# om-ai-lab/OmChat

Measured on AMD Instinct MI355X. Metric: images/sec prefill + decode tokens/sec, OmChat-13B TP=1/8; p50 TTFT, higher is better.
Workload: dtype bf16

## Files before the change

### include/omchat_hip.h

```cpp
#ifndef OMCHAT_HIP_H
#define OMCHAT_HIP_H
#include <stddef.h>
#include <stdint.h>

#ifdef __cplusplus
extern "C" {
#endif

#define OMCHAT_F16 0
#define OMCHAT_BF16 1
#define OMCHAT_F32 2
#define OMCHAT_PAD_ROW INT32_MIN

typedef struct omchat_ctx omchat_ctx;

typedef struct {
  int v_hidden;
  int v_heads;
  int v_qk_channels;
  int v_mlp;
  int v_layers;
  int v_patch;
  int v_image;
  float v_eps;
// ... 58 lines not shown
#define OMCHAT_CON_MAX_SUPPRESS 1024
#define OMCHAT_CON_MAX_BAD_WORDS 1024
#define OMCHAT_CON_MAX_BAD_WORD_IDS 8192
int omchat_set_constraints(omchat_ctx* ctx, int b, int no_repeat_ngram_size, int min_new_tokens, int min_length, const int32_t* eos_ids, int n_eos,
                           const int32_t* suppress_ids, int n_suppress, const int32_t* begin_suppress_ids, int n_begin_suppress,
                           const int32_t* bad_word_ids, const int32_t* bad_word_offsets, int n_bad_words, const int32_t* prompt_ids,
                           const int32_t* prompt_len, int max_new, void* stream);
#define OMCHAT_FSM_MAX_STATES (1 << 20)
#define OMCHAT_FSM_MAX_EDGES (1 << 26)
#define OMCHAT_FSM_DEAD (-1)
int omchat_fsm_load(omchat_ctx* ctx, int n_states, const int32_t* off, const int32_t* tok, const int32_t* nxt, void* stream);
int omchat_fsm_begin(omchat_ctx* ctx, int b, const int32_t* start_states, int max_new, void* stream);
int omchat_fsm_states(omchat_ctx* ctx, int b, int32_t* out, void* stream);
int omchat_set_guidance(omchat_ctx* ctx, int b, float scale, void* stream);
#define OMCHAT_DOLA_MAX_LAYERS 16
int omchat_set_dola(omchat_ctx* ctx, int b, const int32_t* layers, int k, float relative_top, int norm, void* stream);
int omchat_dola_read(omchat_ctx* ctx, int32_t* out, int rows, int steps);
int omchat_dola_rows(omchat_ctx* ctx, float* out);
int omchat_set_logprobs(omchat_ctx* ctx, int b, int max_new, void* stream);
int omchat_read_logprobs(omchat_ctx* ctx, int b, float* raw, float* processed, int32_t* counts, int max_len);
#define OMCHAT_LP_MAX_TOP 20
#define OMCHAT_LP_MAX_SCORED 32
int omchat_set_logprobs_ex(omchat_ctx* ctx, int b, int max_new, int top_n, const int32_t* score_ids, int n_score, void* stream);
int omchat_read_logprob_extras(omchat_ctx* ctx, int b, float* top_vals, int32_t* top_ids, float* scored, int32_t* counts, int max_len);
int omchat_read_sampling_state(omchat_ctx* ctx, int row, int* step, uint32_t* seen_words);
int omchat_kv_lengths(omchat_ctx* ctx, int32_t* out, int b);
int omchat_kv_rewind(omchat_ctx* ctx, int b, int n, void* stream);

int omchat_beam_begin(omchat_ctx* ctx, int b, int num_beams, float length_penalty, int early_stopping, const int32_t* eos_ids, int n_eos,
                      int max_new, int prompt_tok_len, void* stream);
int omchat_beam_step(omchat_ctx* ctx, const float* logits, int rows, int32_t* next_tokens, int32_t* done_word, void* stream);
int omchat_beam_result(omchat_ctx* ctx, int num_return, int32_t* tokens, int32_t* lengths, float* scores, int max_len);

int omchat_group_begin(omchat_ctx* ctx, int b, int N, int prompt_len, int share, void* stream);
int omchat_group_share_available(omchat_ctx* ctx, int N);

#define OMCHAT_VERIFY_KEEP_ALL 1
#define OMCHAT_VERIFY_SAMPLE 2
int omchat_decode_verify(omchat_ctx* ctx, const int32_t* tokens, int T, float* logits, int32_t* picks,
                         int* n_accept, int flags, void* stream);

int omchat_prefill_extend(omchat_ctx* ctx, const void* embeds, int S_new, int keep, float* logits_last, void* hidden_out, void* stream);
int omchat_extend_attn_form(int S_new, int keep, int Hkv);
int omchat_kv_read(omchat_ctx* ctx, int layer, int which, int pos0, int n, void* out, void* stream);
int omchat_kv_read_row(omchat_ctx* ctx, int row, int layer, int which, int pos0, int n, void* out, void* stream);

int omchat_prefill_suffixes(omchat_ctx* ctx, const void* embeds, int N, int S_max, const int32_t* lengths, int keep, float* logits_last,
                            void* hidden_out, void* stream);
int omchat_suffix_attn_form(int shared, int n_rep);

int omchat_enable_decode_graph(omchat_ctx* ctx, int on);
int omchat_decode_graph_stats(omchat_ctx* ctx, long* steps, long* replays, long* captures);
int omchat_bf16x12_stats(omchat_ctx* ctx, int* roles, long* launches, int* coded);

int omchat_enable_fp8_decode(omchat_ctx* ctx, int on);

int omchat_enable_mxfp4_decode(omchat_ctx* ctx, int mode);

enum omchat_weight_format {
  OMCHAT_WFMT_16 = 0,
  OMCHAT_WFMT_16_PACKED = 1,
  OMCHAT_WFMT_E4M3 = 2,
  OMCHAT_WFMT_MXFP4 = 3,
  OMCHAT_WFMT_MXFP4_PACKED = 4,
  OMCHAT_WFMT_COUNT = 5
};
int omchat_decode_weight_format(int rows, int fp8_on, int mxfp4_mode, int packed16_ready, int geometry_ok, int* x_pack_nb);

int omchat_enable_fp8_kv(omchat_ctx* ctx, int on);
int omchat_enable_fp8_prefill(omchat_ctx* ctx, int on);

#define OMCHAT_PROF_DECODE_GATEUP 0
#define OMCHAT_PROF_PREFILL_GATEUP 1
#define OMCHAT_PROF_VIT_FC1 2
#define OMCHAT_PROF_CATS 3
int omchat_prof_enable(omchat_ctx* ctx, int on);
int omchat_prof_read(omchat_ctx* ctx, int cat, double* total_ms, long* launches, int reset);

int omchat_mha_fwd(const void* qkv, int B, int S, int H, float softmax_scale, int causal, void* out, int dtype, void* stream);
int omchat_mha_fwd_varlen(const void* qkv, int B, int S, int H, int D, const int32_t* seqlens, float softmax_scale, int causal,
                          void* out, int dtype, void* stream);

int omchat_op_gemm(int dtype, const void* A, int lda, const void* W, int ldw, void* C, int ldc, int M, int N, int K,
                   const void* bias, const void* ls, const void* resid, int ldr, int epi, int force_tile, void* stream);
int omchat_op_gemm_fused(int dtype, const void* A, int lda, const void* W, int ldw, void* C, int ldc, int M, int N, int K,
                         const void* bias, const void* ls, const void* resid, int ldr, int epi, int force_tile, const float* row_scale,
                         const float* rs_stats, int rs_ld, int rs_nslots, int rs_dim, float rs_eps,
                         float* stats, int stats_ld, int* nslots, void* stream);
int omchat_op_stats_finish(const float* stats, int ld, int slot0, int nslots, int ngroups, int rows, int dim, float eps, float* out, void* stream);
int omchat_op_row_sumsq(int dtype, const void* x, int ldx, int rows, int H, float* stats, void* stream);
int omchat_op_fold_cols(int dtype, const void* W, const void* n, void* out, int rows, int cols, void* stream);
int omchat_op_vit_knorm_slots(int dtype, void* k, int ld, const void* wk, int rows, int C, int C_total, float eps, const float* stats, int stats_ld,
                              int nslots, float* sumsq_q, void* stream);
int omchat_op_mha_qnorm(int dtype, const void* qkv, int B, int Sq, int H, const float* sumsq, int stride, int dim, const void* wq,
                        float eps, float q_scale, void* out, void* stream);
int omchat_op_gemv_norm(int dtype, const void* X, const void* W, int ldw, void* Y, int N, int K, const void* norm_w, float eps,
                        const void* bias, int epi, int out_f32, void* stream);
int omchat_op_set_tuning(int key, int value);
int omchat_gemm_tune_load(const char* path);
int omchat_gemm_tune_dump(const char* path);
long omchat_gemm_tune_runs(void);
size_t omchat_op_gemm_sk_ws(void);
int omchat_op_gemm_sk(int dtype, const void* A, int lda, const void* W, int ldw, void* C, int ldc, int M, int N, int K,
                      const void* bias, const void* ls, const void* resid, int ldr, int epi, int force_tile, void* ws,
                      size_t ws_bytes, int stream_k, void* stream);
int omchat_op_gemv(int dtype, const void* X, int ldx, const void* W, int ldw, void* Y, int ldy, int b, int N, int K,
                   const void* bias, const void* resid, int ldr, int epi, int out_f32, void* stream);
int omchat_op_gemv_packed(int dtype, const void* X, int ldx, const void* W, int ldw, void* Y, int ldy, int b, int N, int K,
                          const void* bias, int epi, int out_f32, int ksplit, int w_packed, int y_packed, void* stream);
int omchat_op_pack_x(int dtype, const void* X, int ldx, int b, int K, void* out, void* stream);
#define OMCHAT_GEMV_PLAN_INTS 20
int omchat_op_gemv_plan(int dtype, int b, int N, int K, int epi, int ksplit, int flags, int wf, int n_cu, int* out);
int omchat_op_gemv_split_k(int b, int K, int H, int packed, int down);
int omchat_op_gemm_fp8(int dtype, const void* A8, const float* a_scale, const void* W8, const float* w_scale, void* C, int ldc, int M, int N,
                       int K, const void* bias, const void* resid, int ldr, int epi, void* stream);
int omchat_op_quant_rows_fp8(int dtype, const void* x, const void* norm_w, float eps, void* y8, float* scale, int rows, int H, void* stream);
int omchat_op_quant_fp8(int dtype, const void* W, int N, int K, void* W8, float* scale, void* stream);
int omchat_op_gemv_fp8(int dtype, const void* X, const void* W8, const float* scale, void* Y, int N, int K, const void* bias,
                       const void* resid, int epi, int out_f32, int ksplit, void* stream);
int omchat_op_quant_mxfp4(int dtype, const void* W, int N, int K, void* W4, void* S, void* stream);
int omchat_op_gemv_mxfp4(int dtype, const void* X, const void* W4, const void* S, void* Y, int N, int K, const void* bias,
                         const void* resid, int epi, int out_f32, int ksplit, void* stream);
int omchat_op_gemv_mxfp4_norm(int dtype, const void* X, const void* W4, const void* S, void* Y, int N, int K, const void* norm_w, float eps,
                              const void* bias, int epi, int out_f32, void* stream);
int omchat_op_gemv_mxfp4_rows(int dtype, const void* X, int ldx, const void* W4, const void* S, void* Y, int ldy, int b, int N, int K,
                              const void* bias, int epi, int out_f32, int ksplit, void* stream);
int omchat_op_gemv_mxfp4_packed(int dtype, const void* X, int ldx, const void* W4, const void* S, void* Y, int ldy, int b, int N, int K,
                                const void* bias, int epi, int out_f32, int ksplit, int y_packed, void* stream);
int omchat_op_encode_bf16x12(const void* W, int N, int K, void* coded, void* top, void* cnt, void* patch, void* over, void* stream);
int omchat_op_gemv_bf16x12(const void* X, const void* coded, const void* top, const void* cnt, const void* patch, void* Y, int N, int K,
                           const void* norm_w, float eps, const void* resid, int epi, int out_f32, void* stream);
int omchat_op_pack_w(int dtype, const void* W, int ldw, int N, int K, void* out, void* stream);
int omchat_op_pack_w4(const void* W4, const void* S, int N, int K, void* W4P, void* SP, void* stream);
int omchat_op_gemv_prepacked(int dtype, const void* XP, const void* WP, const void* SP, void* Y, int ldy, int b, int N, int K, const void* bias,
                             int epi, int out_f32, int ksplit, int y_packed, void* stream);
int omchat_op_rmsnorm(int dtype, const void* x, const void* w, void* y, int rows, int H, float eps, void* stream);
int omchat_op_resid_rmsnorm(int dtype, void* x, int ldx, const float* part, int ks, const void* w, void* xn, int ldn, int rows, int H,
                            float eps, int pack_nb, void* stream);
int omchat_op_vit_qknorm(int dtype, void* qkv, int ld, const void* wq, const void* wk, int rows, int C, int C_total,
                         float eps, float q_scale, void* stream);
int omchat_op_attn_prefill(int dtype, const void* q, const void* k, const void* v, void* out, int b, int Sq, int Skv,
                           int Hq, int Hkv, const int32_t* kv_len, int causal, int q_pos0, float scale, void* stream);
int omchat_op_attn_prefill_d(int dtype, const void* q, const void* k, const void* v, void* out, int b, int Sq, int Skv,
                             int Hq, int Hkv, int D, const int32_t* kv_len, int causal, int q_pos0, float scale, void* stream);
int omchat_op_layernorm(int dtype, const void* x, const void* w, const void* b, void* y, int rows, int H, float eps, void* stream);
size_t omchat_op_attn_decode_ws(int b, int Hq, int L);
int omchat_op_attn_decode(int dtype, const void* q, const void* k, const void* v, void* out, int b, int Hq, int Hkv,
                          int cap, int L, const int32_t* kv_len, float scale, void* ws, size_t ws_bytes, void* stream);
int omchat_op_attn_verify(int dtype, const void* q, void* k, void* v, void* out, int T, int Hq, int Hkv, int cap, int L, float scale,
                          void* ws, size_t ws_bytes, void* stream);
int omchat_op_attn_verify_tpw(int keys, int Hkv);
size_t omchat_op_attn_extend_ws(int Sq, int Hq, int Hkv, int L);
int omchat_op_attn_extend(int dtype, const void* q, const void* k, const void* v, void* out, int Sq, int Hq, int Hkv, int cap, int L,
                          float scale, void* ws, size_t ws_bytes, void* stream);
size_t omchat_op_attn_shared_ws(int G, int N, int Hq, int Hkv, int P, int L);
int omchat_op_attn_shared(int dtype, const void* q, void* k, void* v, void* out, int G, int N, int Hq, int Hkv, int cap, int P, int L,
                          float scale, void* ws, size_t ws_bytes, void* stream);
int omchat_op_attn_shared_lens(int dtype, const void* q, void* k, void* v, void* out, int G, int N, int Hq, int Hkv, int cap, int P, int L,
                               const int* kv_len, float scale, void* ws, size_t ws_bytes, void* stream);
size_t omchat_op_attn_suffix_ws(int N, int S, int Hq, int Hkv, int P);
int omchat_op_attn_suffix(int dtype, const void* q, const void* k, const void* v, void* out, int N, int S, int Hq, int Hkv, int cap, int P,
                          const int32_t* lengths, int* kv_len_dev, float scale, void* ws, size_t ws_bytes, void* stream);
int omchat_op_attn_verify_append(int dtype, const void* qkv, float theta, void* k, void* v, void* out, int T, int Hq, int Hkv, int cap,
                                 int L, float scale, void* ws, size_t ws_bytes, void* stream);
int omchat_op_attn_decode_kv8(int dtype, const void* q, const void* k8, const void* v8, const float* ks, const float* vs, void* out, int b,
                              int Hq, int Hkv, int cap, int L, const int32_t* kv_len, float scale, void* ws, size_t ws_bytes, void* stream);
int omchat_op_attn_decode_kv8_masked(int dtype, const void* q, const void* k8, const void* v8, const float* ks, const float* vs, void* out, int b,
                                     int Hq, int Hkv, int cap, int L, const unsigned char* key_mask, int64_t mask_sb, float scale, void* ws,
                                     size_t ws_bytes, void* stream);
int omchat_op_attn_merge(int dtype, const float* ws, int nsplit, int q_heads, int rows, const int32_t* kv_len, int L, float scale, void* out,
                         int split_keys, void* stream);
int omchat_op_kv_quant(int dtype, const void* k16, const void* v16, void* k8, void* v8, float* ks, float* vs, int b, int Hkv, int cap,
                       const int32_t* pos_lo, int pos0, const int32_t* len, int max_rows, void* stream);
int omchat_op_attn_decode_kv8_append(int dtype, void* qkv, float theta, void* k8, void* v8, float* ks, float* vs, void* k16, void* v16, void* out,
                                     int b, int Hq, int Hkv, int cap, int L, const int32_t* kv_len, const int32_t* pos, float scale, void* ws,
                                     size_t ws_bytes, void* stream);
int omchat_op_rope_kv(int dtype, void* qkv, int b, int S, int Hq, int Hkv, int pos0, float theta, void* kcache, void* vcache,
                      int cap, void* stream);
int omchat_op_rope_kv_q8(int dtype, void* qkv, int b, int S, int Hq, int Hkv, int pos0, float theta, void* kcache, void* vcache, int cap,
                         void* k8, void* v8, float* ks, float* vs, void* stream);
int omchat_op_argmax(const float* logits, int b, int V, int32_t* out, void* stream);
int omchat_op_attn_prefill_left(int dtype, const void* q, const void* k, const void* v, void* out, int b, int Sq, int Skv, int Hq, int Hkv,
                                const int32_t* kv_len, const int32_t* kv_start, int causal, int q_pos0, float scale, int fill_uniform, void* stream);
int omchat_op_rope_kv_pos(int dtype, void* qkv, int b, int S, int Hq, int Hkv, const int32_t* pos, int pos0, int slot0, int max_pos, float theta,
// ... 99 lines not shown
```

### omchat_amd/_lib.py

```python
import ctypes as C
import os

HERE = os.path.dirname(os.path.abspath(__file__))
LIB_PATH = os.environ.get("OMCHAT_LIB") or os.path.join(HERE, "lib", "libomchat_hip.so")
_lib = None

F16, BF16, F32 = 0, 1, 2
EPI_NONE, EPI_GELU, EPI_LS_RESID, EPI_RESID, EPI_SWIGLU = 0, 1, 2, 3, 4
EPI_F32OUT = 6
EPI_LS_RESID_STATS, EPI_NONE_STATS = 7, 8
PAD_ROW = -(2 ** 31)
PROF_DECODE_GATEUP, PROF_PREFILL_GATEUP, PROF_VIT_FC1 = 0, 1, 2


class OmchatConfig(C.Structure):
    _fields_ = [
        ("v_hidden", C.c_int), ("v_heads", C.c_int), ("v_qk_channels", C.c_int), ("v_mlp", C.c_int), ("v_layers", C.c_int),
        ("v_patch", C.c_int), ("v_image", C.c_int), ("v_eps", C.c_float),
        ("t_hidden", C.c_int), ("t_layers", C.c_int), ("t_heads", C.c_int), ("t_kv_heads", C.c_int), ("t_mlp", C.c_int),
        ("t_vocab", C.c_int), ("t_vocab_total", C.c_int), ("t_eps", C.c_float), ("rope_theta", C.c_float),
        ("max_seq", C.c_int), ("max_batch", C.c_int), ("max_tiles", C.c_int), ("max_prefill_rows", C.c_int), ("dtype", C.c_int),
        ("v_head_dim", C.c_int), ("v_norm_type", C.c_int), ("v_no_qk_norm", C.c_int),
    ]

# ... 39 lines not shown
    "omchat_dola_rows": (_i, [_vp, _vp]),
    "omchat_op_dola_ws": (_sz, [_i, _i, _i]),
    "omchat_op_dola": (_i, [_vp, _i, _i, _i, _i, _f, _vp, _i, _vp, _vp, _sz, _vp]),
    "omchat_kv_lengths": (_i, [_vp, _vp, _i]),
    "omchat_kv_rewind": (_i, [_vp, _i, _i, _vp]),
    "omchat_set_logprobs": (_i, [_vp, _i, _i, _vp]),
    "omchat_read_logprobs": (_i, [_vp, _i, _vp, _vp, _vp, _i]),
    "omchat_set_logprobs_ex": (_i, [_vp, _i, _i, _i, _vp, _i, _vp]),
    "omchat_read_logprob_extras": (_i, [_vp, _i, _vp, _vp, _vp, _vp, _i]),
    "omchat_group_begin": (_i, [_vp, _i, _i, _i, _i, _vp]),
    "omchat_group_share_available": (_i, [_vp, _i]),
    "omchat_beam_begin": (_i, [_vp, _i, _i, _f, _i, _vp, _i, _i, _i, _vp]),
    "omchat_beam_step": (_i, [_vp, _vp, _i, _vp, _vp, _vp]),
    "omchat_beam_result": (_i, [_vp, _i, _vp, _vp, _vp, _i]),
    "omchat_decode_verify": (_i, [_vp, _vp, _i, _vp, _vp, _vp, _i, _vp]),
    "omchat_decode_step_masked": (_i, [_vp, _vp, _i, _vp, _vp, _i, _vp, _vp, _vp]),
    "omchat_masked_decode_begin": (_i, [_vp, _i, _vp, _vp, _i, _i, _vp]),
    "omchat_decode_step_masked_next": (_i, [_vp, _vp, _i, _vp, _vp, _vp]),
    "omchat_fused_status": (_i, [_vp, C.POINTER(C.c_long), C.POINTER(C.c_uint)]),
    "omchat_has_experiments": (_i, []),
    "omchat_set_allreduce_hook": (_i, [_vp, _vp, _vp]),
    "omchat_allreduce_noop": (_i, [_vp, _vp, C.c_size_t, _i, _vp]),
    "omchat_op_gemv_norm": (_i, [_i, _vp, _vp, _i, _vp, _i, _i, _vp, _f, _vp, _i, _i, _vp]),
    "omchat_prof_enable": (_i, [_vp, _i]),
    "omchat_prof_read": (_i, [_vp, _i, C.POINTER(C.c_double), C.POINTER(C.c_long), _i]),
    "omchat_mha_fwd": (_i, [_vp, _i, _i, _i, _f, _i, _vp, _i, _vp]),
    "omchat_mha_fwd_varlen": (_i, [_vp, _i, _i, _i, _i, _vp, _f, _i, _vp, _i, _vp]),
    "omchat_op_gemm": (_i, [_i, _vp, _i, _vp, _i, _vp, _i, _i, _i, _i, _vp, _vp, _vp, _i, _i, _i, _vp]),
    "omchat_op_gemm_fused": (_i, [_i, _vp, _i, _vp, _i, _vp, _i, _i, _i, _i, _vp, _vp, _vp, _i, _i, _i, _vp, _vp, _i, _i, _i, _f, _vp, _i, _vp, _vp]),
    "omchat_op_stats_finish": (_i, [_vp, _i, _i, _i, _i, _i, _i, _f, _vp, _vp]),
    "omchat_op_row_sumsq": (_i, [_i, _vp, _i, _i, _i, _vp, _vp]),
    "omchat_op_fold_cols": (_i, [_i, _vp, _vp, _vp, _i, _i, _vp]),
    "omchat_op_vit_knorm_slots": (_i, [_i, _vp, _i, _vp, _i, _i, _i, _f, _vp, _i, _i, _vp, _vp]),
    "omchat_op_mha_qnorm": (_i, [_i, _vp, _i, _i, _i, _vp, _i, _i, _vp, _f, _f, _vp, _vp]),
    "omchat_ctx_sp_stats": (_i, [_vp, C.POINTER(C.c_long), C.POINTER(C.c_long)]),
    "omchat_op_set_tuning": (_i, [_i, _i]),
    "omchat_gemm_tune_load": (_i, [C.c_char_p]),
    "omchat_gemm_tune_dump": (_i, [C.c_char_p]),
    "omchat_gemm_tune_runs": (C.c_long, []),
    "omchat_op_gemm_sk_ws": (_sz, []),
    "omchat_op_gemm_sk": (_i, [_i, _vp, _i, _vp, _i, _vp, _i, _i, _i, _i, _vp, _vp, _vp, _i, _i, _i, _vp, _sz, _i, _vp]),
    "omchat_op_gemv": (_i, [_i, _vp, _i, _vp, _i, _vp, _i, _i, _i, _i, _vp, _vp, _i, _i, _i, _vp]),
    "omchat_op_gemv_packed": (_i, [_i, _vp, _i, _vp, _i, _vp, _i, _i, _i, _i, _vp, _i, _i, _i, _i, _i, _vp]),
    "omchat_op_pack_x": (_i, [_i, _vp, _i, _i, _i, _vp, _vp]),
    "omchat_op_gemv_plan": (_i, [_i, _i, _i, _i, _i, _i, _i, _i, _i, _vp]),
    "omchat_op_gemv_split_k": (_i, [_i, _i, _i, _i, _i]),
    "omchat_op_gemm_fp8": (_i, [_i, _vp, _vp, _vp, _vp, _vp, _i, _i, _i, _i, _vp, _vp, _i, _i, _vp]),
    "omchat_op_quant_rows_fp8": (_i, [_i, _vp, _vp, _f, _vp, _vp, _i, _i, _vp]),
    "omchat_enable_fp8_decode": (_i, [_vp, _i]),
    "omchat_enable_fp8_kv": (_i, [_vp, _i]),
    "omchat_enable_fp8_prefill": (_i, [_vp, _i]),
    "omchat_enable_decode_graph": (_i, [_vp, _i]),
    "omchat_bf16x12_stats": (_i, [_vp, C.POINTER(_i), C.POINTER(C.c_long), C.POINTER(_i)]),
    "omchat_decode_graph_stats": (_i, [_vp, C.POINTER(C.c_long), C.POINTER(C.c_long), C.POINTER(C.c_long)]),
    "omchat_op_quant_fp8": (_i, [_i, _vp, _i, _i, _vp, _vp, _vp]),
    "omchat_op_gemv_fp8": (_i, [_i, _vp, _vp, _vp, _vp, _i, _i, _vp, _vp, _i, _i, _i, _vp]),
    "omchat_enable_mxfp4_decode": (_i, [_vp, _i]),
    "omchat_decode_weight_format": (_i, [_i, _i, _i, _i, _i, C.POINTER(_i)]),
    "omchat_op_quant_mxfp4": (_i, [_i, _vp, _i, _i, _vp, _vp, _vp]),
    "omchat_op_gemv_mxfp4": (_i, [_i, _vp, _vp, _vp, _vp, _i, _i, _vp, _vp, _i, _i, _i, _vp]),
    "omchat_op_gemv_mxfp4_rows": (_i, [_i, _vp, _i, _vp, _vp, _vp, _i, _i, _i, _i, _vp, _i, _i, _i, _vp]),
    "omchat_op_gemv_mxfp4_packed": (_i, [_i, _vp, _i, _vp, _vp, _vp, _i, _i, _i, _i, _vp, _i, _i, _i, _i, _vp]),
    "omchat_op_pack_w": (_i, [_i, _vp, _i, _i, _i, _vp, _vp]),
    "omchat_op_pack_w4": (_i, [_vp, _vp, _i, _i, _vp, _vp, _vp]),
    "omchat_op_gemv_prepacked": (_i, [_i, _vp, _vp, _vp, _vp, _i, _i, _i, _i, _vp, _i, _i, _i, _i, _vp]),
    "omchat_op_encode_bf16x12": (_i, [_vp, _i, _i, _vp, _vp, _vp, _vp, _vp, _vp]),
    "omchat_op_gemv_bf16x12": (_i, [_vp, _vp, _vp, _vp, _vp, _vp, _i, _i, _vp, _f, _vp, _i, _i, _vp]),
    "omchat_op_gemv_mxfp4_norm": (_i, [_i, _vp, _vp, _vp, _vp, _i, _i, _vp, _f, _vp, _i, _i, _vp]),
    "omchat_op_rmsnorm": (_i, [_i, _vp, _vp, _vp, _i, _i, _f, _vp]),
    "omchat_op_resid_rmsnorm": (_i, [_i, _vp, _i, _vp, _i, _vp, _vp, _i, _i, _i, _f, _i, _vp]),
    "omchat_op_vit_qknorm": (_i, [_i, _vp, _i, _vp, _vp, _i, _i, _i, _f, _f, _vp]),
    "omchat_op_attn_prefill": (_i, [_i, _vp, _vp, _vp, _vp, _i, _i, _i, _i, _i, _vp, _i, _i, _f, _vp]),
    "omchat_op_attn_prefill_d": (_i, [_i, _vp, _vp, _vp, _vp, _i, _i, _i, _i, _i, _i, _vp, _i, _i, _f, _vp]),
    "omchat_op_layernorm": (_i, [_i, _vp, _vp, _vp, _vp, _i, _i, _f, _vp]),
    "omchat_op_attn_decode_ws": (_sz, [_i, _i, _i]),
    "omchat_op_attn_decode": (_i, [_i, _vp, _vp, _vp, _vp, _i, _i, _i, _i, _i, _vp, _f, _vp, _sz, _vp]),
    "omchat_op_attn_verify_tpw": (_i, [_i, _i]),
    "omchat_op_attn_verify": (_i, [_i, _vp, _vp, _vp, _vp, _i, _i, _i, _i, _i, _f, _vp, _sz, _vp]),
    "omchat_op_attn_extend_ws": (_sz, [_i, _i, _i, _i]),
    "omchat_op_attn_shared_ws": (_sz, [_i, _i, _i, _i, _i, _i]),
    "omchat_op_attn_shared": (_i, [_i, _vp, _vp, _vp, _vp, _i, _i, _i, _i, _i, _i, _i, _f, _vp, _sz, _vp]),
    "omchat_op_attn_extend": (_i, [_i, _vp, _vp, _vp, _vp, _i, _i, _i, _i, _i, _f, _vp, _sz, _vp]),
    "omchat_prefill_extend": (_i, [_vp, _vp, _i, _i, _vp, _vp, _vp]),
    "omchat_extend_attn_form": (_i, [_i, _i, _i]),
    "omchat_kv_read": (_i, [_vp, _i, _i, _i, _i, _vp, _vp]),
    "omchat_kv_read_row": (_i, [_vp, _i, _i, _i, _i, _i, _vp, _vp]),
    "omchat_prefill_suffixes": (_i, [_vp, _vp, _i, _i, _vp, _i, _vp, _vp, _vp]),
    "omchat_suffix_attn_form": (_i, [_i, _i]),
    "omchat_op_attn_shared_lens": (_i, [_i, _vp, _vp, _vp, _vp, _i, _i, _i, _i, _i, _i, _i, _vp, _f, _vp, _sz, _vp]),
    "omchat_op_attn_suffix_ws": (_sz, [_i, _i, _i, _i, _i]),
    "omchat_op_attn_suffix": (_i, [_i, _vp, _vp, _vp, _vp, _i, _i, _i, _i, _i, _i, _vp, _vp, _f, _vp, _sz, _vp]),
    "omchat_op_attn_verify_append": (_i, [_i, _vp, _f, _vp, _vp, _vp, _i, _i, _i, _i, _i, _f, _vp, _sz, _vp]),
    "omchat_op_attn_decode_kv8": (_i, [_i, _vp, _vp, _vp, _vp, _vp, _vp, _i, _i, _i, _i, _i, _vp, _f, _vp, _sz, _vp]),
    "omchat_op_attn_decode_kv8_masked": (_i, [_i, _vp, _vp, _vp, _vp, _vp, _vp, _i, _i, _i, _i, _i, _vp, _i64, _f, _vp, _sz, _vp]),
    "omchat_op_attn_merge": (_i, [_i, _vp, _i, _i, _i, _vp, _i, _f, _vp, _i, _vp]),
    "omchat_op_kv_quant": (_i, [_i, _vp, _vp, _vp, _vp, _vp, _vp, _i, _i, _i, _vp, _i, _vp, _i, _vp]),
    "omchat_op_attn_decode_kv8_append": (_i, [_i, _vp, _f, _vp, _vp, _vp, _vp, _vp, _vp, _vp, _i, _i, _i, _i, _i, _vp, _vp, _f, _vp, _sz, _vp]),
    "omchat_op_attn_decode_append": (_i, [_i, _vp, _f, _vp, _vp, _vp, _i, _i, _i, _i, _i, _vp, _vp, _vp, _i64, _i, _f, _vp, _sz, _vp]),
    "omchat_op_rope_kv": (_i, [_i, _vp, _i, _i, _i, _i, _i, _f, _vp, _vp, _i, _vp]),
    "omchat_op_rope_kv_q8": (_i, [_i, _vp, _i, _i, _i, _i, _i, _f, _vp, _vp, _i, _vp, _vp, _vp, _vp, _vp]),
    "omchat_op_argmax": (_i, [_vp, _i, _i, _vp, _vp]),
    "omchat_op_attn_prefill_left": (_i, [_i, _vp, _vp, _vp, _vp, _i, _i, _i, _i, _i, _vp, _vp, _i, _i, _f, _i, _vp]),
    "omchat_op_rope_kv_pos": (_i, [_i, _vp, _i, _i, _i, _i, _vp, _i, _i, _i, _f, _vp, _vp, _i, _vp]),
    "omchat_op_argmax_ld": (_i, [_vp, _i, _i, _i, _vp, _vp, _vp, _vp]),
    "omchat_op_im2col": (_i, [_i, _vp, _vp, _i, _i, _i, _i, _vp]),
    "omchat_op_vit_assemble": (_i, [_i, _vp, _vp, _vp, _vp, _i, _i, _i, _vp]),
    "omchat_op_gather_rows": (_i, [_i, _vp, _vp, _vp, _vp, _i, _i, _vp]),
    "omchat_op_copy_rows": (_i, [_i, _vp, _i64, _vp, _i64, _i, _i, _i, _i, _vp]),
    "omchat_op_tp_finish": (_i, [_i, _vp, _vp, _vp, _vp, _vp, _i, _i, _i, _vp]),
    "omchat_op_resid16_norm": (_i, [_i, _vp, _i, _vp, _i, _vp, _vp, _vp, _i, _i, _i, _f, _vp]),
    "omchat_op_cast_f32": (_i, [_i, _vp, _vp, _i64, _vp]),
    "omchat_op_rmsnorm_ld": (_i, [_i, _vp, _i, _vp, _vp, _i, _i, _i, _f, _i, _vp]),
    "omchat_op_layernorm_ld": (_i, [_i, _vp, _i, _vp, _vp, _vp, _i, _i, _i, _f, _vp]),
    "omchat_op_sample": (_i, [_vp, _i, _i, _u64, _f, _i, C.c_double, _f, _vp, _vp, _i, _vp, _vp, _vp]),
    "omchat_op_token_logprob": (_i, [_vp, _i, _i, _i, _vp, _vp, _f, _f, _vp, _vp, _vp, _vp, _vp, _vp, _vp]),
    "omchat_op_lse_label_ws": (_sz, [_i, _i]),
    "omchat_op_lse_label": (_i, [_i, _vp, _i, _vp, _i, _i, _i, _i, _vp, _vp, _vp, _vp, _sz, _vp]),
    "omchat_op_top_logprobs": (_i, [_vp, _i, _i, _i, _i, _vp, _i, _vp, _vp, _vp, _vp]),
    "omchat_op_sample_filtered": (_i, [_vp, _i, _i, _u64, _f, _i, C.c_double, _f, C.c_double, C.c_double, C.c_double, C.c_double, _vp, _vp, _i,
                                       _vp, _vp, _vp, _vp]),
# ... 87 lines not shown
```

### omchat_amd/csrc/capi.hip

```cpp
#include "kernels.h"
#include <stdlib.h>
#include "../../include/omchat_hip.h"
#include <math.h>
#include <vector>

#define S(x) ((hipStream_t)(x))
#if OMCHAT_EXPERIMENTS
int g_launch_any_order = 0;
#endif

extern "C" int omchat_op_gemm(int dtype, const void* A, int lda, const void* W, int ldw, void* C, int ldc, int M, int N, int K,
                              const void* bias, const void* ls, const void* resid, int ldr, int epi, int force_tile, void* stream) {
  GemmArgs g{A, lda, W, ldw, C, ldc, M, N, K, bias, ls, resid, ldr, epi, force_tile, nullptr, 0, -1};
  return launch_gemm(dtype, g, S(stream));
}

extern "C" int omchat_op_gemm_fused(int dtype, const void* A, int lda, const void* W, int ldw, void* C, int ldc, int M, int N, int K,
                                    const void* bias, const void* ls, const void* resid, int ldr, int epi, int force_tile, const float* row_scale,
                                    const float* rs_stats, int rs_ld, int rs_nslots, int rs_dim, float rs_eps,
                                    float* stats, int stats_ld, int* nslots, void* stream) {
  GemmArgs g{A, lda, W, ldw, C, ldc, M, N, K, bias, ls, resid, ldr, epi, force_tile, nullptr, 0, -1};
  g.row_scale = row_scale; g.stats = stats; g.stats_ld = stats_ld; g.stats_nslots = nslots;
  g.rs_stats = rs_stats; g.rs_ld = rs_ld; g.rs_nslots = rs_nslots; g.rs_dim = rs_dim; g.rs_eps = rs_eps;
  return launch_gemm(dtype, g, S(stream));
// ... 21 lines not shown
  a.V = (const char*)qkv + (size_t)2 * H * 128 * 2; a.v_sb = a.q_sb; a.v_sh = 128; a.v_sr = row;
  a.O = out; a.o_sb = (int64_t)Sq * H * 128; a.o_sh = 128; a.o_sr = (int64_t)H * 128;
  a.batch = B; a.q_heads = H; a.kv_heads = H; a.Sq = Sq; a.Skv = Sq; a.kv_len = nullptr; a.causal = 0; a.q_pos0 = 0;
  a.scale = 1.0f;
  a.qn_sumsq = sumsq; a.qn_stride = stride; a.qn_dim = dim; a.qn_w = wq; a.qn_eps = eps; a.qn_scale = q_scale;
  return launch_attn_prefill(dtype, a, S(stream));
}

extern "C" int omchat_op_set_tuning(int key, int value) {
  const char* allow = getenv("OMCHAT_ALLOW_TUNING");
  if (!allow || allow[0] != '1') {
    omchat_set_error("omchat_op_set_tuning: process-global test / measurement hook; set OMCHAT_ALLOW_TUNING=1 to use it (see include/omchat_hip.h)");
    return 1;
  }
  if (key == 0) { gemm_set_skew(value); return 0; }
  if (key == 1) { gemv_set_force_mfma(value); return 0; }
  if (key == 5) { gemm_set_autotune(value); return 0; }
  if (key == 4) { model_set_ar_min_rows(value); return 0; }
  if (key == 6) { model_set_pack_replica(value); return 0; }
  if (key == 8) { attn_set_v2(value); return 0; }
  if (key == 9) { model_set_fuse_peer_norm(value); return 0; }
  if (key == 10) { attn_set_tpw(value); return 0; }
  if (key == 11) { gemv_set_no_xs(value); return 0; }
  if (key == 12) { attn_set_klds(value); return 0; }
  if (key == 25) { attn_set_dma(value); return 0; }
  if (key == 26) { attn_set_dma_slots(value); return 0; }
  if (key == 27) { attn_set_dma_rot(value); return 0; }
  if (key == 28) { gemv_set_skew(value); return 0; }
  if (key == 29) { model_set_tp_f32(value); return 0; }
  if (key == 30) { attn_set_hsplit(value); return 0; }
  if (key == 33) { attn_set_mha_xcd(value); return 0; }
  if (key == 16) { gemv_set_norm_loop(value); return 0; }
  if (key == 17) { gemv_set_rows_balance(value); return 0; }
  if (key == 19) { attn_set_merge_mid_min(value); return 0; }
  if (key == 21) { attn_set_merge_dg(value); return 0; }
  if (key == 13) { gemm_set_persist(value); return 0; }
  if (key == 14) { model_set_norm_in_gemv(value); return 0; }
  if (key == 22) { model_set_fuse_attn_oproj(value); return 0; }
  if (key == 23) { model_set_decode_layer(value); return 0; }
  if (key == 24) { gemv_set_dyn(value); return 0; }
  if (key == 34) { gemv_set_shard_shapes(value); return 0; }
  if (key == 35) { model_set_shard_as_tp1(value); return 0; }
  if (key == 36) { attn_set_kg(value); return 0; }
  if (key == 37) { gemm_set_wide_store(value); return 0; }
  if (key == 43) { gemm_set_skip_dead(value); return 0; }
  if (key == 44) { model_set_vit_fused(value); return 0; }
  if (key == 45) { model_set_tp_sp(value); return 0; }
  if (key == 46) { attn_set_peel(value); return 0; }
  if (key == 47) { attn_set_kv8_tpw(value); return 0; }
  if (key == 48) { attn_set_kv8_fuse(value); return 0; }
  if (key == 49) { model_set_extend_attn(value); return 0; }
  if (key == 50) { model_set_x12_roles(value); return 0; }
  if (key == 51) { model_set_suffix_attn(value); return 0; }
  if (key == 38) { gemv_set_gu_rr(value); return 0; }
  if (key == 39) { gemv_set_longk_direct(value); return 0; }
  if (key == 40) { norm_set_wave(value); return 0; }
#if OMCHAT_EXPERIMENTS
  if (key == 41) { g_launch_any_order = value; return 0; }
  if (key == 42) { model_set_ao_oproj(value); return 0; }
#endif
  omchat_set_error("omchat_op_set_tuning: unknown key");
  return 1;
}

extern "C" int omchat_allreduce_noop(void*, void*, size_t, int, void*) { return 0; }

extern "C" int omchat_gemm_tune_load(const char* path) { OM_CHECK(path, "null path"); return gemm_tune_load(path); }
extern "C" int omchat_gemm_tune_dump(const char* path) { OM_CHECK(path, "null path"); return gemm_tune_dump(path); }
extern "C" long omchat_gemm_tune_runs(void) { return gemm_tune_runs(); }

extern "C" size_t omchat_op_gemm_sk_ws(void) { return gemm_sk_ws_bytes(); }

extern "C" int omchat_op_gemm_sk(int dtype, const void* A, int lda, const void* W, int ldw, void* C, int ldc, int M, int N, int K,
                                 const void* bias, const void* ls, const void* resid, int ldr, int epi, int force_tile, void* ws,
                                 size_t ws_bytes, int stream_k, void* stream) {
  GemmArgs g{A, lda, W, ldw, C, ldc, M, N, K, bias, ls, resid, ldr, epi, force_tile, ws, ws_bytes, stream_k};
  return launch_gemm(dtype, g, S(stream));
}

extern "C" int omchat_op_gemv(int dtype, const void* X, int ldx, const void* W, int ldw, void* Y, int ldy, int b, int N, int K,
                              const void* bias, const void* resid, int ldr, int epi, int out_f32, void* stream) {
  GemvArgs g{X, ldx, W, ldw, Y, ldy, b, N, K, bias, resid, ldr, epi, out_f32};
  return launch_gemv(dtype, g, S(stream));
}

extern "C" int omchat_op_gemv_norm(int dtype, const void* X, const void* W, int ldw, void* Y, int N, int K, const void* norm_w, float eps,
                                   const void* bias, int epi, int out_f32, void* stream) {
  OM_CHECK(X && W && Y && norm_w, "null argument");
  GemvArgs g{X, K, W, ldw, Y, N, 1, N, K, bias, nullptr, 0, epi, out_f32};
  g.norm_w = norm_w; g.norm_eps = eps;
  return launch_gemv(dtype, g, S(stream));
}

extern "C" int omchat_op_gemv_packed(int dtype, const void* X, int ldx, const void* W, int ldw, void* Y, int ldy, int b, int N, int K,
                                     const void* bias, int epi, int out_f32, int ksplit, int w_packed, int y_packed, void* stream) {
  OM_CHECK(b >= 1 && b <= 32 && K % 64 == 0, "1 <= b <= 32, K % 64 == 0");
  const int NB = b > 16 ? 2 : 1;
  void *xp = nullptr, *wp = nullptr;
  OM_HIP(hipMalloc(&xp, (size_t)NB * 16 * K * 2));
  int rc = launch_pack_x(dtype, X, ldx, b, K, xp, S(stream));
  if (rc == 0 && w_packed) {
    if (hipMalloc(&wp, (size_t)N * K * 2) != hipSuccess) { hipFree(xp); omchat_set_error("hipMalloc failed"); return 2; }
    rc = launch_pack_w(dtype, W, ldw, N, K, wp, S(stream));
  }
  if (rc == 0) {
    GemvArgs g{xp, K, w_packed ? wp : W, ldw, Y, ldy, b, N, K, bias, nullptr, 0, epi, out_f32, ksplit, 0, nullptr, 1, w_packed, y_packed};
    rc = launch_gemv(dtype, g, S(stream));
  }
  hipStreamSynchronize(S(stream));
  hipFree(xp); if (wp) hipFree(wp);
  return rc;
}
extern "C" int omchat_op_pack_x(int dtype, const void* X, int ldx, int b, int K, void* out, void* stream) { return launch_pack_x(dtype, X, ldx, b, K, out, S(stream)); }

extern "C" int omchat_op_gemv_plan(int dtype, int b, int N, int K, int epi, int ksplit, int flags, int wf, int n_cu, int* out) {
  OM_CHECK(out && wf >= WF_16 && wf <= WF_X12, "null out or weight form outside 0..3");
  static const unsigned set[1] = {0};
  GemvArgs a{};
  a.b = b; a.N = N; a.K = K; a.epi = epi; a.ksplit = ksplit;
  a.ldx = K; a.ldy = a.ldr = N; a.ldw = wf == WF_MX4 ? K / 2 : wf == WF_X12 ? K / 2 * 3 : K;
  a.x_packed = flags & 1; a.w_packed = flags >> 1 & 1; a.y_packed = flags >> 2 & 1; a.out_f32 = flags >> 4 & 1; a.force_mfma = flags >> 5 & 1;
  if (flags & 8) a.norm_w = set;
  if (flags & 64) a.resid = set;
  if (wf == WF_E4M3) a.w_scale = (const float*)set;
  if (wf == WF_MX4) a.mx_scale = (const unsigned char*)set;
  if (wf == WF_X12) { a.x12_top = a.x12_cnt = (const unsigned char*)set; a.x12_patch = set; }
  const GemvPlan g = gemv_plan(dtype, a, gemv_tuning(), n_cu > 0 ? n_cu : device_cus());
  if (g.refusal) { omchat_set_error(g.refusal); return 1; }
  const int f[OMCHAT_GEMV_PLAN_INTS] = {g.family, g.wf, g.wpack, g.epi, g.ntile, g.waves, g.unroll, g.nb, g.rr, g.nch, g.norm, g.gx, g.gy, g.block, g.lds,
                                        g.per_wg, (int)g.skew, g.rows_per_wg, g.n5, g.xskew};
  for (int i = 0; i < OMCHAT_GEMV_PLAN_INTS; ++i) out[i] = f[i];
  return 0;
}
extern "C" int omchat_op_gemv_split_k(int b, int K, int H, int packed, int down) { return gemv_split_k(b, K, H, packed != 0, down != 0, gemv_tuning()); }

extern "C" int omchat_op_gemm_fp8(int dtype, const void* A8, const float* a_scale, const void* W8, const float* w_scale, void* C, int ldc, int M,
                                  int N, int K, const void* bias, const void* resid, int ldr, int epi, void* stream) {
  GemmArgs g{A8, K, W8, K, C, ldc, M, N, K, bias, nullptr, resid, ldr, epi, 0, nullptr, 0, -1, 1, a_scale, w_scale};
  return launch_gemm(dtype, g, S(stream));
}
extern "C" int omchat_op_quant_rows_fp8(int dtype, const void* x, const void* norm_w, float eps, void* y8, float* scale, int rows, int H, void* stream) {
  if (norm_w) return launch_rmsnorm_q8(dtype, x, H, norm_w, y8, H, scale, rows, H, eps, S(stream));
  return launch_quant_rows_q8(dtype, x, H, y8, H, scale, rows, H, S(stream));
}

extern "C" int omchat_op_resid_rmsnorm(int dtype, void* x, int ldx, const float* part, int ks, const void* w, void* xn, int ldn, int rows, int H,
                                       float eps, int pack_nb, void* stream) {
  OM_CHECK(x && part, "null argument");
  return launch_resid_rmsnorm(dtype, x, ldx, part, ks, w, xn, ldn, rows, H, eps, S(stream), pack_nb);
}
extern "C" int omchat_op_rmsnorm(int dtype, const void* x, const void* w, void* y, int rows, int H, float eps, void* stream) {
  return launch_rmsnorm(dtype, x, H, w, y, H, rows, H, eps, S(stream));
}

extern "C" int omchat_op_vit_qknorm(int dtype, void* qkv, int ld, const void* wq, const void* wk, int rows, int C, int C_total, float eps,
                                    float q_scale, void* stream) {
  return launch_vit_qknorm(dtype, qkv, ld, wq, wk, rows, C, C_total, eps, q_scale, nullptr, S(stream));
}

extern "C" int omchat_op_attn_prefill(int dtype, const void* q, const void* k, const void* v, void* out, int b, int Sq, int Skv, int Hq,
                                      int Hkv, const int32_t* kv_len, int causal, int q_pos0, float scale, void* stream) {
  AttnArgs a{};
  a.Q = q; a.q_sb = (int64_t)Sq * Hq * 128; a.q_sh = 128; a.q_sr = (int64_t)Hq * 128;
  a.K = k; a.k_sb = (int64_t)Hkv * Skv * 128; a.k_sh = (int64_t)Skv * 128; a.k_sr = 128;
  a.V = v; a.v_sb = a.k_sb; a.v_sh = a.k_sh; a.v_sr = 128;
  a.O = out; a.o_sb = a.q_sb; a.o_sh = 128; a.o_sr = a.q_sr;
  a.batch = b; a.q_heads = Hq; a.kv_heads = Hkv; a.Sq = Sq; a.Skv = Skv; a.kv_len = kv_len; a.causal = causal; a.q_pos0 = q_pos0; a.scale = scale;
  return launch_attn_prefill(dtype, a, S(stream));
}

extern "C" size_t omchat_op_attn_decode_ws(int b, int Hq, int L) { return attn_decode_ws_bytes(b, Hq, L); }

static void bind_dense(AttnOperands& a, const void* q, bool qkv_rows, const void* k, const void* v, void* out, int Hq, int Hkv, int cap, float scale,
                       void* ws, size_t ws_bytes) {
  a.Q = q; a.q_sb = (int64_t)(qkv_rows ? Hq + 2 * Hkv : Hq) * 128; a.q_sh = 128;
  a.K = k; a.k_sb = (int64_t)Hkv * cap * 128; a.k_sh = (int64_t)cap * 128; a.k_sr = 128;
  a.V = v; a.v_sb = a.k_sb; a.v_sh = a.k_sh; a.v_sr = 128;
  a.O = out; a.o_sb = (int64_t)Hq * 128; a.o_sh = 128;
  a.q_heads = Hq; a.kv_heads = Hkv; a.scale = scale; a.ws = (float*)ws; a.ws_bytes = ws_bytes;
// ... 706 lines not shown
  const int NB = b > 16 ? 2 : 1;
  void *xp = nullptr, *wp = nullptr, *sp = nullptr;
  auto drop = [&]() { if (xp) hipFree(xp); if (wp) hipFree(wp); if (sp) hipFree(sp); };
  if (hipMalloc(&xp, (size_t)NB * 16 * K * 2) != hipSuccess || hipMalloc(&wp, (size_t)N * (K / 2)) != hipSuccess ||
      hipMalloc(&sp, (size_t)N * (K / 32)) != hipSuccess) {
    (void)hipGetLastError(); drop(); omchat_set_error("hipMalloc failed"); return 2;
  }
  int rc = launch_pack_x(dtype, X, ldx, b, K, xp, S(stream));
  if (rc == 0) rc = launch_pack_w4(W4, (const unsigned char*)S_, N, K, wp, (unsigned char*)sp, S(stream));
  if (rc == 0) {
    GemvArgs g{xp, K, wp, K / 2, Y, ldy, b, N, K, bias, nullptr, 0, epi, out_f32, ksplit, 0, nullptr, 1, 1, y_packed};
    g.mx_scale = (const unsigned char*)sp;
    rc = launch_gemv(dtype, g, S(stream));
  }
  hipStreamSynchronize(S(stream));
  drop();
  return rc;
}

extern "C" int omchat_op_pack_w(int dtype, const void* W, int ldw, int N, int K, void* out, void* stream) { return launch_pack_w(dtype, W, ldw, N, K, out, S(stream)); }
extern "C" int omchat_op_pack_w4(const void* W4, const void* S_, int N, int K, void* W4P, void* SP, void* stream) {
  return launch_pack_w4(W4, (const unsigned char*)S_, N, K, W4P, (unsigned char*)SP, S(stream));
}
extern "C" int omchat_op_gemv_prepacked(int dtype, const void* XP, const void* WP, const void* SP, void* Y, int ldy, int b, int N, int K, const void* bias,
                                        int epi, int out_f32, int ksplit, int y_packed, void* stream) {
  OM_CHECK(XP && WP && Y, "null argument");
  OM_CHECK(b >= 1 && b <= 32 && K >= 64 && K % 64 == 0 && N >= 16 && N % 16 == 0, "pre-packed GEMV: 1 <= b <= 32, K % 64 == 0, N % 16 == 0");
  GemvArgs g{XP, K, WP, SP ? K / 2 : K, Y, ldy, b, N, K, bias, nullptr, 0, epi, out_f32, ksplit, 0, nullptr, 1, 1, y_packed};
  g.mx_scale = (const unsigned char*)SP;
  return launch_gemv(dtype, g, S(stream));
}

extern "C" int omchat_op_gemv_mxfp4_norm(int dtype, const void* X, const void* W4, const void* S_, void* Y, int N, int K, const void* norm_w,
                                         float eps, const void* bias, int epi, int out_f32, void* stream) {
  OM_CHECK(X && W4 && S_ && Y && norm_w, "null argument");
  OM_CHECK(K % 32 == 0, "MXFP4: K must be a multiple of 32 (one e8m0 scale per 32 consecutive k)");
  GemvArgs g{X, K, W4, K / 2, Y, N, 1, N, K, bias, nullptr, 0, epi, out_f32};
  g.norm_w = norm_w; g.norm_eps = eps;
  g.mx_scale = (const unsigned char*)S_;
  return launch_gemv(dtype, g, S(stream));
}

extern "C" int omchat_op_encode_bf16x12(const void* W, int N, int K, void* coded, void* top, void* cnt, void* patch, void* over, void* stream) {
  return launch_encode_bf16x12(W, K, N, K, coded, (unsigned char*)top, (unsigned char*)cnt, (unsigned*)patch, (int*)over, S(stream));
}
extern "C" int omchat_op_gemv_bf16x12(const void* X, const void* coded, const void* top, const void* cnt, const void* patch, void* Y, int N, int K,
                                      const void* norm_w, float eps, const void* resid, int epi, int out_f32, void* stream) {
  OM_CHECK(X && coded && top && cnt && patch && Y, "null argument");
  GemvArgs g{X, K, coded, K / 2 * 3, Y, N, 1, N, K, nullptr, resid, N, epi, out_f32};
  g.norm_w = norm_w; g.norm_eps = eps;
  g.x12_top = (const unsigned char*)top; g.x12_cnt = (const unsigned char*)cnt; g.x12_patch = (const unsigned*)patch;
  return launch_gemv(OMCHAT_BF16, g, S(stream));
}

extern "C" int omchat_op_attn_prefill_d(int dtype, const void* q, const void* k, const void* v, void* out, int b, int Sq, int Skv, int Hq,
                                        int Hkv, int D, const int32_t* kv_len, int causal, int q_pos0, float scale, void* stream) {
  AttnArgs a{};
  a.Q = q; a.q_sb = (int64_t)Sq * Hq * D; a.q_sh = D; a.q_sr = (int64_t)Hq * D;
  a.K = k; a.k_sb = (int64_t)Hkv * Skv * D; a.k_sh = (int64_t)Skv * D; a.k_sr = D;
  a.V = v; a.v_sb = a.k_sb; a.v_sh = a.k_sh; a.v_sr = D;
  a.O = out; a.o_sb = a.q_sb; a.o_sh = D; a.o_sr = a.q_sr;
  a.batch = b; a.q_heads = Hq; a.kv_heads = Hkv; a.Sq = Sq; a.Skv = Skv; a.kv_len = kv_len; a.causal = causal; a.q_pos0 = q_pos0; a.scale = scale;
  a.head_dim = D;
  return launch_attn_prefill(dtype, a, S(stream));
}

extern "C" int omchat_op_layernorm(int dtype, const void* x, const void* w, const void* b, void* y, int rows, int H, float eps, void* stream) {
  return launch_layernorm(dtype, x, H, w, b, y, H, rows, H, eps, S(stream));
}

extern "C" int omchat_op_attn_prefill_left(int dtype, const void* q, const void* k, const void* v, void* out, int b, int Sq, int Skv, int Hq,
                                           int Hkv, const int32_t* kv_len, const int32_t* kv_start, int causal, int q_pos0, float scale,
                                           int fill_uniform, void* stream) {
  OM_CHECK(q && k && v && out && kv_start, "null argument");
  AttnArgs a{};
  a.Q = q; a.q_sb = (int64_t)Sq * Hq * 128; a.q_sh = 128; a.q_sr = (int64_t)Hq * 128;
  a.K = k; a.k_sb = (int64_t)Hkv * Skv * 128; a.k_sh = (int64_t)Skv * 128; a.k_sr = 128;
  a.V = v; a.v_sb = a.k_sb; a.v_sh = a.k_sh; a.v_sr = 128;
  a.O = out; a.o_sb = a.q_sb; a.o_sh = 128; a.o_sr = a.q_sr;
  a.batch = b; a.q_heads = Hq; a.kv_heads = Hkv; a.Sq = Sq; a.Skv = Skv; a.kv_len = kv_len; a.kv_start = kv_start; a.causal = causal;
  a.q_pos0 = q_pos0; a.scale = scale;
  int rc = launch_attn_prefill(dtype, a, S(stream));
  if (!rc && fill_uniform) rc = launch_attn_uniform_rows(dtype, a, S(stream));
  return rc;
}

extern "C" int omchat_op_rope_kv_pos(int dtype, void* qkv, int b, int Sq, int Hq, int Hkv, const int32_t* pos, int pos0, int slot0, int max_pos,
                                     float theta, void* kcache, void* vcache, int cap, void* stream) {
  OM_CHECK(qkv && kcache && vcache && b >= 1 && Sq >= 1 && Hq >= 1 && Hkv >= 1 && max_pos >= 1 && cap >= 1 && slot0 >= -1, "bad argument");
  if (pos) {
    std::vector<int32_t> hp((size_t)b * Sq);
    OM_HIP(hipStreamSynchronize(S(stream)));
    OM_HIP(hipMemcpy(hp.data(), pos, hp.size() * 4, hipMemcpyDeviceToHost));
    for (int32_t p : hp) {
      OM_CHECK(p >= 0 && p < max_pos, "position outside the RoPE table");
      OM_CHECK(slot0 >= 0 || p < cap, "cache slot exceeds the capacity");
    }
  } else {
    OM_CHECK(pos0 >= 0 && pos0 + Sq <= max_pos, "position outside the RoPE table");
    OM_CHECK(slot0 >= 0 || pos0 + Sq <= cap, "cache slot exceeds the capacity");
  }
  OM_CHECK(slot0 < 0 || slot0 + Sq <= cap, "cache slot exceeds the capacity");
  float* d = rope_table_device(max_pos, theta);
  OM_CHECK(d, "rope table allocation failed");
  RopeArgs r{qkv, (Hq + 2 * Hkv) * 128, b * Sq, Sq, Hq, Hkv, pos, pos0, d, max_pos, kcache, vcache, (int64_t)Hkv * cap * 128, (int64_t)cap * 128};
  r.slot0 = slot0;
// ... 57 lines not shown
```

### omchat_amd/csrc/ctx.h

```cpp
#pragma once
#include "kernels.h"
#include "../../include/omchat_hip.h"
#include <rccl/rccl.h>
#include <algorithm>
#include <string>
#include <unordered_map>
#include <vector>

#define TRY(x) do { int rc_ = (x); if (rc_) return rc_; } while (0)

extern int g_fuse_peer_norm;

enum RouteKind { R_PLAIN = 0, R_GATE = 1, R_UP = 2, R_PATCH = 3 };
struct Route {
  void* dst = nullptr;
  int64_t rows = 0, cols = 0;
  int64_t dst_ld = 0;
  int kind = R_PLAIN;
  bool loaded = false;
  float synth_std = 0.02f, synth_off = 0.f;
};

struct Grown {
  void* p = nullptr; size_t cap = 0;
// ... 77 lines not shown
  bool dola_fresh = false;
  bool dola_on() const { return dola.on; }
  bool guidance_on() const { return gd.on; }
  int pick_rows(int rows) const { return gd.on ? rows / 2 : rows; }
  bool sampling_on() const { return smp.on; }
  bool constraints_on() const { return con.on; }
  bool logprobs_on() const { return lp.on; }
  bool fsm_on() const { return fsm.on; }
  void release() { con_hist.release(); lp_rec.release(); lp_xrec.release(); fsm_mem.release(); fsm_trail.release(); dola_rec.release(); }
};

struct BeamState {
  struct Search { bool on = false; int b = 0, N = 0, KB = 0, max_new = 0, P = 0, es = 0, ns = 1, t = 0; float lp = 1.f; std::vector<int> eos; };
  Search cur;
  Grown state, table, dn, parents, stash;
  bool stash8 = false;
  std::vector<int> hpos, hlen;
  bool on() const { return cur.on; }
  void end() { cur.on = false; }
  void release() { for (Grown* g : {&state, &table, &dn, &parents, &stash}) g->release(); }
};

struct GroupState {
  bool share = false; int b = 0, N = 0, P = 0;
  Grown ws;
  std::vector<int> hpos, hlen;
  bool on() const { return share; }
  void end() { share = false; }
  void release() { ws.release(); }
};

struct omchat_ctx {
  omchat_config c;
  int dt = OMCHAT_BF16;
  int tp_rank = 0, tp_size = 1;
  ncclComm_t comm = nullptr;
  std::vector<void*> allocs;
  size_t bytes = 0;
  std::unordered_map<std::string, Route> routes;

  int v_np = 0, v_ntok = 0, v_Cq = 0, v_kpad = 0, v_hd = 128;
  int t_qdim = 0, t_kvdim = 0, t_qkvdim = 0;

  struct VitLayer { void *ls1, *ls2, *n1, *n2, *n1b, *n2b, *wqkv, *qn, *kn, *wproj, *bproj, *w1, *b1, *w2, *b2; };
  struct DecLayer { void *ln1, *ln2, *wqkv, *bqkv, *wo, *wgu, *wd; };
  enum Proj { P_QKV = 0, P_O = 1, P_GU = 2, P_DOWN = 3, P_LM = 4 };
  struct WRef { void* W = nullptr; int ldw = 0; float* w_scale = nullptr; unsigned char* mx_scale = nullptr; int packed = 0; };
  enum WState { W_ABSENT = 0, W_BUILT, W_STALE, W_UNAVAILABLE };
  struct WTable { std::vector<WRef> e; int state = W_ABSENT; };
  WTable wt[OMCHAT_WFMT_COUNT];
  const WRef* layer_w(int fmt, int layer) const { return &wt[fmt].e[(size_t)layer * 4]; }
  const WRef& lm_w(int fmt) const { return wt[fmt].e.back(); }
  bool built(int fmt) const { return wt[fmt].state == W_BUILT; }
  enum X12Role { X12_GU = 0, X12_DOWN = 1, X12_LM = 2, X12_ROLES = 3 };
  struct X12Ref { void* W = nullptr; unsigned char* top = nullptr; unsigned char* cnt = nullptr; unsigned* patch = nullptr; bool ok = false; };
  struct X12Table { std::vector<X12Ref> e; int state = W_ABSENT; };
  X12Table x12[X12_ROLES];
  int* x12_over = nullptr;
  long x12_launches[X12_ROLES] = {0, 0, 0};
  bool fp8_decode = false;
  int mxfp4_mode = 0;
  void *k8cache = nullptr, *v8cache = nullptr;
  float *ks8 = nullptr, *vs8 = nullptr;
  bool fp8_kv = false, kv8_valid = false, fp8_prefill = false;
  void* tw_q8 = nullptr; float* tw_q8s = nullptr;
  int64_t scale_layer_stride() const { return (int64_t)c.max_batch * c.t_kv_heads * c.max_seq; }
  struct DecodeGraph { hipGraph_t graph = nullptr; hipGraphExec_t exec = nullptr; int cap_len = 0, grp_N = 0, grp_P = 0; const void* grp_ws = nullptr; };
  std::unordered_map<int, DecodeGraph> graphs;
  bool graph_on = false;
  hipStream_t graph_stream = nullptr;
  hipEvent_t graph_ev_in = nullptr, graph_ev_out = nullptr;
  int32_t *d_tok_in = nullptr, *d_tok_out = nullptr;
  long graph_steps = 0, graph_replays = 0, graph_captures = 0;
  void *v_cls = nullptr, *v_pos = nullptr, *v_wpatch = nullptr, *v_bpatch = nullptr;
  std::vector<VitLayer> vl;
  void *p_w0 = nullptr, *p_b0 = nullptr, *p_w2 = nullptr, *p_b2 = nullptr;
  void *t_embed = nullptr, *t_norm = nullptr, *t_lm = nullptr;
  std::vector<DecLayer> dl;
  float* rope = nullptr;

  void *vw_cols = nullptr, *vw_pe = nullptr, *vw_x = nullptr, *vw_x2 = nullptr, *vw_xn = nullptr, *vw_qkv = nullptr, *vw_ao = nullptr,
       *vw_h = nullptr, *vw_feat = nullptr, *vw_proj = nullptr;
  float* vw_sumsq = nullptr;
  float *vw_stats_x = nullptr, *vw_stats_qk = nullptr, *vw_rstd = nullptr;
  int vw_stats_x_ld = 0, vw_stats_qk_ld = 0, vw_stats_x_ld_used = 1;
  struct VitFold { void *wqkv = nullptr, *w1 = nullptr; };
  std::vector<VitFold> vfold;
  bool vfold_stale = true;
  void *tw_x = nullptr, *tw_x2 = nullptr, *tw_xn = nullptr, *tw_qkv = nullptr, *tw_ao = nullptr, *tw_act = nullptr, *tw_last = nullptr;
  float* tw_logits = nullptr;
  void* sk_ws = nullptr; size_t sk_ws_bytes = 0;
  float* tp_f32_ws = nullptr; size_t tp_f32_bytes = 0;
  float* tw_part = nullptr;
  float* tw_attn_ws = nullptr;
  size_t tw_attn_ws_bytes = 0;
  void* fd_ws = nullptr;
  unsigned* fd_err = nullptr;
  unsigned fd_epoch = 0;
  long n_fused_launches = 0;
  void* dl_ws = nullptr;
  long n_layer_launches = 0;
  unsigned long long* dbg_stamps = nullptr;
  unsigned* dyn_ctr = nullptr;
  int *d_pos = nullptr, *d_len = nullptr, *d_idx = nullptr, *d_start = nullptr;
  int* d_verify_n = nullptr;
  PickState pick;
  BeamState beam;
  GroupState group;
  Grown ext_ws;
  Grown score_ws;
  int grow(Grown& g, size_t n) {
    if (n <= g.cap) return 0;
// ... 170 lines not shown
```

### omchat_amd/csrc/gemv.hip

```cpp
#include "kernels.h"
#include "rowdot.h"
#include <type_traits>

namespace {

struct GemvP {
  const void* X; const void* W; void* Y; const void* bias; const void* resid;
  int ldx, ldw, ldy, ldr, b, N, K, out_f32, ksplit;
  const float* w_scale;
  int y_packed;
  const void* norm_w; float norm_eps;
  unsigned* dyn;
  void* y_pack;
  unsigned long long* dbg;
  const unsigned char* mx_s;
  const unsigned char* x12_top;
  const unsigned char* x12_cnt;
  const unsigned* x12_patch;
#if OMCHAT_EXPERIMENTS
  int xskew;
#endif
};
#if OMCHAT_EXPERIMENTS
#define OM_DBG_MIN(slot, cond) do { if (p.dbg && (cond) && threadIdx.x == 0) atomicMax(p.dbg + (slot), ~wall_clock64()); } while (0)
// ... 650 lines not shown
  s.pv = p.x12_patch[row * 32 + (lane & 31)];
}
__device__ __forceinline__ void x12_row_finish(X12Row& s) {
  const int t = __builtin_amdgcn_readfirstlane((int)s.top_raw) - 7;
  s.cnt = __builtin_amdgcn_readfirstlane((int)s.cnt_raw);
  s.pi = 0;
  s.tlo = ((unsigned)((t + 1) & 0x7f) << 8) | ((unsigned)((t + 2) & 0x7f) << 16) | ((unsigned)((t + 3) & 0x7f) << 24);
  s.thi = (unsigned)((t + 4) & 0x7f) | ((unsigned)((t + 5) & 0x7f) << 8) | ((unsigned)((t + 6) & 0x7f) << 16) | ((unsigned)((t + 7) & 0x7f) << 24);
}
__device__ __forceinline__ rw_u32x4 x12_decode(const X12W& w, const X12Row& s) {
  const unsigned n = w.nib;
  const unsigned c0 = n & 0x07070707u, c1 = (n >> 4) & 0x07070707u;
  unsigned h0 = __builtin_amdgcn_perm(s.thi, s.tlo, c0), h1 = __builtin_amdgcn_perm(s.thi, s.tlo, c1);
  h0 |= (n & 0x08080808u) << 4;
  h1 |= n & 0x80808080u;
  rw_u32x4 r;
  r.x = __builtin_amdgcn_perm(h0, w.lo.x, 0x05010400u);
  r.y = __builtin_amdgcn_perm(h0, w.lo.x, 0x07030602u);
  r.z = __builtin_amdgcn_perm(h1, w.lo.y, 0x05010400u);
  r.w = __builtin_amdgcn_perm(h1, w.lo.y, 0x07030602u);
  return r;
}
__device__ __forceinline__ void x12_apply(rw_u32x4& w, unsigned e, int lane) {
  const unsigned k = e >> 16, i = k & 7u, sh = (i & 1u) * 16u;
  const unsigned keep = ~(0xffffu << sh), ins = (e & 0xffffu) << sh;
  const bool mine = lane == (int)((k >> 3) & 63u);
  w.x = (mine && (i >> 1) == 0u) ? ((w.x & keep) | ins) : w.x;
  w.y = (mine && (i >> 1) == 1u) ? ((w.y & keep) | ins) : w.y;
  w.z = (mine && (i >> 1) == 2u) ? ((w.z & keep) | ins) : w.z;
  w.w = (mine && (i >> 1) == 3u) ? ((w.w & keep) | ins) : w.w;
}
template <int G>
__device__ __forceinline__ void x12_group(rw_u32x4 (&wd)[G], const X12W* w, X12Row& s, int chunk0, int nch, int lane) {
#pragma unroll
  for (int i = 0; i < G; ++i) wd[i] = x12_decode(w[i], s);
  while (s.pi < s.cnt) {
    const unsigned e = (unsigned)__builtin_amdgcn_readlane((int)s.pv, s.pi);
    const int ch = (int)(e >> 25) - chunk0;
    if (ch >= G) break;
#pragma unroll
    for (int i = 0; i < G; ++i) if (ch == i) x12_apply(wd[i], e, lane);
    ++s.pi;
  }
  if (chunk0 + G > nch) {
    for (int j = 0; j < s.cnt; ++j) {
      const unsigned e = (unsigned)__builtin_amdgcn_readlane((int)s.pv, j);
      if ((e >> 19) != 0u) break;
#pragma unroll
      for (int i = 0; i < G; ++i) if (chunk0 + i >= nch) x12_apply(wd[i], e, 0);
    }
  }
}

template <typename T, int WF>
__device__ __forceinline__ typename RwW<WF>::type rw_ldw(const GemvP& p, size_t row, int k) {
  if constexpr (WF == WF_X12) return x12_ldw(p, row, k >> 9, (k >> 3) & 63); else
  if constexpr (WF == WF_E4M3) {
    return __builtin_nontemporal_load(reinterpret_cast<const rw_u32x2*>((const unsigned char*)p.W + row * p.ldw + k));
  } else if constexpr (WF == WF_MX4) {
    rw_u32x2 w;
    w.x = __builtin_nontemporal_load(reinterpret_cast<const unsigned*>((const unsigned char*)p.W + row * p.ldw + (k >> 1)));
    w.y = __builtin_nontemporal_load(p.mx_s + row * (size_t)(p.K >> 5) + (k >> 5));
    return w;
  } else {
    return __builtin_nontemporal_load(reinterpret_cast<const rw_u32x4*>((const T*)p.W + row * p.ldw + k));
  }
}
template <typename T, int WF>
__device__ __forceinline__ float rw_dotw(typename RwW<WF>::type w, rw_u32x4 x, float acc) {
  if constexpr (WF == WF_E4M3) return rw_dot8_fp8<T>(w, x, acc);
  else if constexpr (WF == WF_MX4) return fmaf(rw_dot8_fp4<T>(w.x, x), mx_scale_of(w.y), acc);
  else return rw_dot8<T>(w, x, acc);
}

template <typename T, int R> struct RwTail { const T* p0; const T* p1; int idx[R]; float v0[R], v1[R]; };
template <typename T, int R> __device__ __forceinline__ void rw_tail_load(RwTail<T, R>& t) {
#pragma unroll
  for (int r = 0; r < R; ++r) { t.v0[r] = tof(t.p0[t.idx[r]]); t.v1[r] = tof(t.p1[t.idx[r]]); }
}
template <typename T, int R, int NCH, int WF>
__device__ __forceinline__ void rw_rows_q(const GemvP& p, const int (&rows)[R], int k0, int lane, const rw_u32x4 (&xr)[RW_MAXC], float (&acc)[R],
                                          RwTail<T, R>& tail) {
  typename RwW<WF>::type w[R][NCH];
#pragma unroll
  for (int r = 0; r < R; ++r)
#pragma unroll
    for (int c = 0; c < NCH; ++c) {
      int k = k0 + c * 512 + lane * 8;
      k = k < p.K ? k : k0;
      w[r][c] = rw_ldw<T, WF>(p, (size_t)rows[r], k);
    }
  float sc[R];
#pragma unroll
  for (int r = 0; r < R; ++r) sc[r] = WF == WF_E4M3 ? p.w_scale[rows[r]] : 1.f;
  rw_tail_load<T, R>(tail);
#pragma unroll
  for (int r = 0; r < R; ++r) {
    float a = 0.f;
#pragma unroll
    for (int c = 0; c < NCH; ++c) a = rw_dotw<T, WF>(w[r][c], xr[c], a);
#pragma unroll
    for (int o = 32; o > 0; o >>= 1) a += __shfl_xor(a, o, 64);
    acc[r] = WF == WF_E4M3 ? a * sc[r] : a;
  }
}

template <typename T, int R, int N, int WF>
__device__ __forceinline__ void rw_dispatch_q(int nch, const GemvP& p, const int (&rows)[R], int k0, int lane, const rw_u32x4 (&xr)[RW_MAXC],
                                              float (&acc)[R], RwTail<T, R>& tail) {
  if constexpr (N > 0) {
    if (nch == N) rw_rows_q<T, R, N, WF>(p, rows, k0, lane, xr, acc, tail);
    else rw_dispatch_q<T, R, N - 1, WF>(nch, p, rows, k0, lane, xr, acc, tail);
  }
}

template <typename T, int R, int NCH>
__device__ __forceinline__ void rw_rows(const T* W, int ldw, const int (&rows)[R], int k0, int K, int lane, const rw_u32x4 (&xr)[RW_MAXC],
                                        float (&acc)[R], RwTail<T, R>& tail) {
  rw_u32x4 w[R][NCH];
#pragma unroll
  for (int r = 0; r < R; ++r)
#pragma unroll
    for (int c = 0; c < NCH; ++c) {
      int k = k0 + c * 512 + lane * 8;
      k = k < K ? k : k0;
      w[r][c] = __builtin_nontemporal_load(reinterpret_cast<const rw_u32x4*>(W + (size_t)rows[r] * ldw + k));
    }
  rw_tail_load<T, R>(tail);
#pragma unroll
  for (int r = 0; r < R; ++r) {
    float a = 0.f;
#pragma unroll
    for (int c = 0; c < NCH; ++c) a = rw_dot8<T>(w[r][c], xr[c], a);
#pragma unroll
    for (int o = 32; o > 0; o >>= 1) a += __shfl_xor(a, o, 64);
    acc[r] = a;
  }
}

template <typename T, int R, int N>
__device__ __forceinline__ void rw_dispatch(int nch, const T* W, int ldw, const int (&rows)[R], int k0, int K, int lane,
                                            const rw_u32x4 (&xr)[RW_MAXC], float (&acc)[R], RwTail<T, R>& tail) {
  if constexpr (N > 0) {
    if (nch == N) rw_rows<T, R, N>(W, ldw, rows, k0, K, lane, xr, acc, tail);
    else rw_dispatch<T, R, N - 1>(nch, W, ldw, rows, k0, K, lane, xr, acc, tail);
  }
}

template <typename T, int EPI, int RR, int WAVES, int F8>
__device__ __forceinline__ void gemv_rows_body(const GemvP& p) {
  constexpr int R = EPI == EPI_SWIGLU ? 2 * RR : RR;
  constexpr int OUT = RR;
  const int lane = threadIdx.x & 63, wave = threadIdx.x >> 6;
  const T* W = (const T*)p.W;
  if constexpr (EPI == EPI_RESID && WAVES == 7) OM_DBG_MIN(1, blockIdx.x < 8);
  const int nch_all = (p.K + 511) / 512;
  const int c_lo = (int)(((long)nch_all * blockIdx.y) / p.ksplit), c_hi = (int)(((long)nch_all * (blockIdx.y + 1)) / p.ksplit);
  const int nch = c_hi - c_lo, k0 = c_lo * 512;
  rw_u32x4 xr[RW_MAXC];
#pragma unroll
  for (int c = 0; c < RW_MAXC; ++c) {
    const int k = k0 + c * 512 + lane * 8;
    rw_u32x4 z = {0u, 0u, 0u, 0u};
    xr[c] = (c < nch && k < p.K) ? *reinterpret_cast<const rw_u32x4*>((const T*)p.X + k) : z;
  }
// ... 7 lines not shown
        int n = g * RR + (r % RR); n = n < n_out ? n : n_out - 1;
        rows[r] = 32 * (n >> 4) + (n & 15) + (r / RR) * 16;
      } else {
        const int n = g * R + r;
        rows[r] = n < p.N ? n : p.N - 1;
      }
    }
    float acc[R];
    RwTail<T, R> tail;
    {
      constexpr bool plain = EPI != EPI_SWIGLU && EPI != EPI_PARTIAL;
      const bool hb = plain && p.bias, hr = EPI == EPI_RESID && !p.out_f32;
      tail.p0 = hb ? (const T*)p.bias : (const T*)p.X;
      tail.p1 = hr ? (const T*)p.resid : (const T*)p.X;
#pragma unroll
      for (int r = 0; r < R; ++r) {
        const int n = g * OUT + r;
        tail.idx[r] = (hb || hr) ? (n < n_out ? n : n_out - 1) : 0;
      }
      if (!hb) tail.p0 = tail.p1;
      if (!hr) tail.p1 = tail.p0;
    }
    if constexpr (F8 != WF_16) rw_dispatch_q<T, R, RW_MAXC, F8>(nch, p, rows, k0, lane, xr, acc, tail);
    else rw_dispatch<T, R, RW_MAXC>(nch, W, p.ldw, rows, k0, p.K, lane, xr, acc, tail);
    if (lane == 0) {
#pragma unroll
      for (int r = 0; r < OUT; ++r) {
        const int n = g * OUT + r;
        if (n >= n_out) continue;
        if constexpr (EPI == EPI_SWIGLU) {
          const float gt = rnd<T>(acc[r]), up = rnd<T>(acc[r + RR]);
          ((T*)p.Y)[n] = fromf<T>(rnd<T>(silu(gt)) * up);
        } else if constexpr (EPI == EPI_PARTIAL) {
          ((float*)p.Y)[(size_t)blockIdx.y * p.ldy + n] = acc[r];
        } else {
          float y = acc[r] + (p.bias ? tail.v0[r] : 0.f);
          if (p.out_f32) ((float*)p.Y)[n] = y;
          else {
            y = rnd<T>(y);
            if constexpr (EPI == EPI_RESID) y = tail.v1[r] + y;
            ((T*)p.Y)[n] = fromf<T>(y);
          }
        }
      }
    }
  }
  if constexpr (EPI == EPI_RESID && WAVES == 7) OM_DBG_MAX(3, (blockIdx.x & 7) == 0);
}

template <typename T, int EPI, int RR = 4, int WAVES = 4, bool F8 = false>
__global__ __launch_bounds__(WAVES * 64) void gemv_rows_kernel(GemvP p) { gemv_rows_body<T, EPI, RR, WAVES, F8 ? WF_E4M3 : WF_16>(p); }
template <typename T, int EPI, int RR, int WAVES>
__global__ __launch_bounds__(WAVES * 64) void gemv_rows_mx4_kernel(GemvP p) { gemv_rows_body<T, EPI, RR, WAVES, WF_MX4>(p); }

template <typename T, int EPI, int RR, int NCH, int F8, int WAVES>
__device__ __forceinline__ void gemv_rows_norm_body(const GemvP& p) {
  typedef typename V8<T>::type v8;
  constexpr int R = EPI == EPI_SWIGLU ? 2 * RR : RR;
  __shared__ __attribute__((aligned(16))) T xs[NCH * 512];
  __shared__ float red[WAVES];
  const int lane = threadIdx.x & 63, wave = __builtin_amdgcn_readfirstlane(threadIdx.x >> 6);
  const int n_out = EPI == EPI_SWIGLU ? p.N / 2 : p.N;
  int g = blockIdx.x * WAVES + wave;
#if OMCHAT_EXPERIMENTS
  if constexpr (EPI == EPI_SWIGLU && RR == 1 && WAVES == 4) {
    if (p.xskew) {
      const int x = blockIdx.x & 7, j = blockIdx.x >> 3;
      const int base = ((n_out + 3) / 4) / 8;
      const int n_x = base + ((x & 1) ? -p.xskew : p.xskew);
      if (j >= n_x) return;
      g = (x * base + ((x & 1) ? p.xskew : 0) + j) * 4 + wave;
    }
  }
#endif
  if constexpr (EPI == EPI_SWIGLU) OM_DBG_MIN(4, blockIdx.x < 8);
  if constexpr (EPI == EPI_NONE) OM_DBG_MIN(8, blockIdx.x < 8);
  static_assert(WAVES >= 4 && NCH <= 8, "sum-of-squares order: four owner waves, up to two chunks each");
  constexpr int MC = (NCH + WAVES - 1) / WAVES;
  constexpr int SC = (NCH + 3) / 4;
  rw_u32x4 xq[MC], nq[MC], sq[SC];
#pragma unroll
  for (int i = 0; i < MC; ++i) {
    const int c = wave + WAVES * i, k = c * 512 + lane * 8;
    const rw_u32x4 z = {0u, 0u, 0u, 0u};
    const bool ok = c < NCH && k < p.K;
    xq[i] = ok ? *reinterpret_cast<const rw_u32x4*>((const T*)p.X + k) : z;
    nq[i] = ok ? *reinterpret_cast<const rw_u32x4*>((const T*)p.norm_w + k) : z;
  }
#pragma unroll
  for (int i = 0; i < SC; ++i) {
    if constexpr (WAVES == 4) {
      sq[i] = xq[i];
    } else {
      const int c = wave + 4 * i, k = c * 512 + lane * 8;
      const rw_u32x4 z = {0u, 0u, 0u, 0u};
      sq[i] = (wave < 4 && c < NCH && k < p.K) ? *reinterpret_cast<const rw_u32x4*>((const T*)p.X + k) : z;
    }
  }
  int rows[R];
#pragma unroll
  for (int r = 0; r < R; ++r) {
    if constexpr (EPI == EPI_SWIGLU) {
      int n = g * RR + (r % RR); n = n < n_out ? n : n_out - 1;
      rows[r] = 32 * (n >> 4) + (n & 15) + (r / RR) * 16;
    } else {
      const int n = g * R + r;
// ... 29 lines not shown
    if constexpr (F8 == WF_E4M3) {
#pragma unroll
      for (int r = 0; r < R; ++r) e_scale[r] = p.w_scale[rows[r]];
    }
  }
  X12Row xst[F8 == WF_X12 ? R : 1];
  if constexpr (F8 == WF_X12) {
#pragma unroll
    for (int r = 0; r < R; ++r) x12_row_load(xst[r], p, (size_t)rows[r], lane);
  }
  __builtin_amdgcn_sched_barrier(0);
  float ss = 0.f;
#pragma unroll
  for (int i = 0; i < SC; ++i) {
    const v8 xv = __builtin_bit_cast(v8, sq[i]);
#pragma unroll
    for (int j = 0; j < 8; ++j) { const float v = tof(xv[j]); ss += v * v; }
  }
#pragma unroll
  for (int o = 32; o > 0; o >>= 1) ss += __shfl_xor(ss, o, 64);
  if (lane == 0 && wave < 4) red[wave] = ss;
  asm volatile("s_waitcnt lgkmcnt(0)" ::: "memory");
  __builtin_amdgcn_s_barrier();
  float tot = red[0];
#pragma unroll
  for (int w = 1; w < 4; ++w) tot += red[w];
  const float inv = rsqrtf(tot / (float)p.K + p.norm_eps);
#pragma unroll
  for (int i = 0; i < MC; ++i) {
    const int c = wave + WAVES * i;
    if (c < NCH) {
      const v8 xv = __builtin_bit_cast(v8, xq[i]), wv = __builtin_bit_cast(v8, nq[i]);
      v8 o;
#pragma unroll
      for (int j = 0; j < 8; ++j) o[j] = fromf<T>(tof(wv[j]) * rnd<T>(tof(xv[j]) * inv));
      *reinterpret_cast<v8*>(xs + c * 512 + lane * 8) = o;
    }
  }
  asm volatile("s_waitcnt lgkmcnt(0)" ::: "memory");
  __builtin_amdgcn_s_barrier();
  rw_u32x4 xr[NCH];
#pragma unroll
  for (int c = 0; c < NCH; ++c) xr[c] = *reinterpret_cast<const rw_u32x4*>(xs + c * 512 + lane * 8);
  __builtin_amdgcn_sched_barrier(0);
  float acc[R];
#pragma unroll
  for (int r = 0; r < R; ++r) {
    float a = 0.f;
    if constexpr (F8 == WF_X12) x12_row_finish(xst[r]);
#pragma unroll
    for (int c = 0; c < NCH; ++c) {
      if constexpr (F8 != WF_X12) a = rw_dotw<T, F8>(w[r][c], xr[c], a);
    }
    if constexpr (F8 == WF_X12) {
      constexpr int G0 = NCH < 4 ? NCH : 4, G1 = NCH - G0;
      {
        rw_u32x4 wd[G0];
        x12_group<G0>(wd, &w[r][0], xst[r], 0, NCH, lane);
#pragma unroll
        for (int c = 0; c < G0; ++c) a = rw_dot8<T>(wd[c], xr[c], a);
      }
      if constexpr (G1 > 0) {
        rw_u32x4 wd[G1];
        x12_group<G1>(wd, &w[r][G0], xst[r], G0, NCH, lane);
#pragma unroll
        for (int c = 0; c < G1; ++c) a = rw_dot8<T>(wd[c], xr[G0 + c], a);
      }
    }
#pragma unroll
    for (int o = 32; o > 0; o >>= 1) a += __shfl_xor(a, o, 64);
    if constexpr (F8 == WF_E4M3) a *= e_scale[r];
    acc[r] = a;
  }
  if (lane == 0) {
#pragma unroll
    for (int r = 0; r < RR; ++r) {
      const int n = g * RR + r;
      if (n >= n_out) continue;
      if constexpr (EPI == EPI_SWIGLU) {
        const float gt = rnd<T>(acc[r]), up = rnd<T>(acc[r + RR]);
        ((T*)p.Y)[n] = fromf<T>(rnd<T>(silu(gt)) * up);
      } else {
        const float y = acc[r] + e_bias[r];
        if (p.out_f32) ((float*)p.Y)[n] = y;
        else ((T*)p.Y)[n] = fromf<T>(y);
      }
    }
  }
  if constexpr (EPI == EPI_SWIGLU) { OM_DBG_MAX(5, blockIdx.x + 64 >= gridDim.x); OM_DBG_MAX(16 + (blockIdx.x & 7), blockIdx.x + 512 >= gridDim.x); }
  if constexpr (EPI == EPI_NONE) OM_DBG_MAX(9, (blockIdx.x & 7) == 0);
}

template <typename T, int EPI, int RR, int NCH, bool F8, int WAVES = 4>
__global__ __launch_bounds__(WAVES * 64) void gemv_rows_norm_kernel(GemvP p) { gemv_rows_norm_body<T, EPI, RR, NCH, F8 ? WF_E4M3 : WF_16, WAVES>(p); }
template <typename T, int EPI, int RR, int NCH, int WAVES = 4>
__global__ __launch_bounds__(WAVES * 64) void gemv_rows_norm_mx4_kernel(GemvP p) { gemv_rows_norm_body<T, EPI, RR, NCH, WF_MX4, WAVES>(p); }
template <typename T, int EPI, int RR, int NCH>
__global__ __launch_bounds__(256) void gemv_rows_norm_x12_kernel(GemvP p) { gemv_rows_norm_body<T, EPI, RR, NCH, WF_X12, 4>(p); }

template <typename T, int EPI, int NCH, int F8>
__device__ __forceinline__ void gemv_rows_norm_loop_body(const GemvP& p, int per_wg, unsigned skew) {
  typedef typename V8<T>::type v8;
  constexpr int R = EPI == EPI_SWIGLU ? 2 : 1;
  __shared__ __attribute__((aligned(16))) T xs[NCH * 512];
  __shared__ float red[4];
  const int lane = threadIdx.x & 63, wave = __builtin_amdgcn_readfirstlane(threadIdx.x >> 6);
  const int n_out = EPI == EPI_SWIGLU ? p.N / 2 : p.N;
  int o0 = blockIdx.x * per_wg, o1 = o0 + per_wg < n_out ? o0 + per_wg : n_out;
  if constexpr (EPI == EPI_SWIGLU) OM_DBG_MIN(4, blockIdx.x < 8);
  if (skew) {
    const int l = blockIdx.x & 7;
    int pre = 0;
    for (int i = 0; i < l; ++i) pre += per_wg + (int)((skew >> (4 * i)) & 15u) - 8;
    o0 = (blockIdx.x >> 3) * 8 * per_wg + pre;
    o1 = o0 + per_wg + (int)((skew >> (4 * l)) & 15u) - 8;
    o1 = o1 < n_out ? o1 : n_out;
  }
  typedef typename RwW<F8>::type wreg_t;
  auto row_of = [&](int n, int r) { return EPI == EPI_SWIGLU ? 32 * (n >> 4) + (n & 15) + r * 16 : n; };
  auto load_w = [&](wreg_t (&w)[R][NCH], int n) {
#pragma unroll
    for (int r = 0; r < R; ++r) {
      const size_t row = (size_t)row_of(n, r);
#pragma unroll
      for (int c = 0; c < NCH; ++c) {
        int k = c * 512 + lane * 8;
        k = k < p.K ? k : 0;
        w[r][c] = rw_ldw<T, F8>(p, row, k);
      }
    }
  };
  wreg_t wa[R][NCH], wb[R][NCH], wc[R][NCH];
  const int u0 = o0 + wave;
  if (u0 < o1) load_w(wa, u0);
  if (u0 + 4 < o1) load_w(wb, u0 + 4);
  if (u0 + 8 < o1) load_w(wc, u0 + 8);
  constexpr int MC = (NCH + 3) / 4;
  rw_u32x4 xq[MC], nq[MC];
#pragma unroll
  for (int i = 0; i < MC; ++i) {
    const int c = wave + 4 * i, k = c * 512 + lane * 8;
    const rw_u32x4 z = {0u, 0u, 0u, 0u};
    const bool ok = c < NCH && k < p.K;
    xq[i] = ok ? *reinterpret_cast<const rw_u32x4*>((const T*)p.X + k) : z;
    nq[i] = ok ? *reinterpret_cast<const rw_u32x4*>((const T*)p.norm_w + k) : z;
  }
  __builtin_amdgcn_sched_barrier(0);
  float ss = 0.f;
#pragma unroll
  for (int i = 0; i < MC; ++i) {
    const v8 xv = __builtin_bit_cast(v8, xq[i]);
// ... 541 lines not shown
    }
  }
  g.block = g.nch = 0;
  return false;
}
}

#define OM_NEED(cond, text) do { if (!(cond)) { g.refusal = text; return g; } } while (0)
GemvPlan gemv_plan(int dtype, const GemvArgs& a, const GemvTuning& t, int n_cu) {
  GemvPlan g{};
  OM_NEED(a.b >= 1 && a.b <= 32, "launch_gemv: batch must be 1..32 per call");
  OM_NEED(!a.x_packed || !a.w_scale, "launch_gemv: packed x: 16-bit or MXFP4 weights");
  OM_NEED(!(a.x_packed && a.mx_scale) || (a.w_packed && a.K % 64 == 0), "launch_gemv: packed x with MXFP4 weights: the packed MXFP4 replica (w_packed), K % 64 == 0");
  OM_NEED(!(a.w_scale && a.mx_scale), "launch_gemv: one weight format per launch: e4m3 (w_scale) or MXFP4 (mx_scale)");
  OM_NEED(!a.w_packed || (a.x_packed && a.N % 16 == 0), "launch_gemv: packed W needs packed x and N % 16 == 0");
  OM_NEED(!a.y_packed || (a.x_packed && a.epi == EPI_SWIGLU), "launch_gemv: packed y: SwiGLU epilogue of the packed kernel only");
  if (a.mx_scale) OM_NEED(a.K % 32 == 0 && a.ldw % 4 == 0 && a.ldx % 8 == 0, "launch_gemv: MXFP4 weights: K % 32 == 0 (one e8m0 scale per 32 k), ldw (bytes) % 4, ldx % 8");
  else OM_NEED(a.K % 64 == 0 && a.ldw % 8 == 0 && a.ldx % 8 == 0, "launch_gemv: K % 64, ldw % 8, ldx % 8");
  OM_NEED((!a.w_scale && !(a.mx_scale && !a.x_packed)) || a.b == 1, "launch_gemv: fp8 / MXFP4 weights: batch 1 only (MXFP4 at b > 1: packed x and the packed MXFP4 replica)");
  OM_NEED(a.epi == EPI_NONE || a.epi == EPI_RESID || a.epi == EPI_SWIGLU || a.epi == EPI_PARTIAL, "launch_gemv: bad epilogue");
  OM_NEED(a.ksplit <= 1 || a.epi == EPI_PARTIAL, "launch_gemv: ksplit > 1 only with EPI_PARTIAL (fp32 slices)");
  OM_NEED(a.ksplit <= (a.K + 63) / 64, "launch_gemv: ksplit exceeds the number of 64-wide K chunks");
  OM_NEED(a.epi != EPI_RESID || a.resid, "launch_gemv: resid missing");
  OM_NEED(a.epi != EPI_SWIGLU || a.N % 32 == 0, "launch_gemv: SwiGLU needs N % 32 == 0");
  OM_NEED(!(a.out_f32 && a.epi != EPI_NONE), "launch_gemv: fp32 output only with EPI_NONE");
  OM_NEED(dtype == OMCHAT_F16 || dtype == OMCHAT_BF16, "launch_gemv: bad dtype");
  const int ks = a.ksplit > 1 ? a.ksplit : 1;
  const bool mfma = a.force_mfma || t.force_mfma;
  g.epi = a.epi; g.gy = 1;
  g.wf = a.x12_top ? WF_X12 : a.mx_scale ? WF_MX4 : a.w_scale ? WF_E4M3 : WF_16;
  OM_NEED(!(a.norm_w && a.x_packed) || (a.w_packed && ks == 1 && (a.K >> 6) == 56 && a.epi == EPI_SWIGLU && a.N % 32 == 0 && !t.no_xs),
          "launch_gemv: the in-register RMSNorm on packed x exists for the x-stationary gate|up form only (packed W, K = 3584, no split-K)");
  OM_NEED(!(a.epi == EPI_RESID && a.x_packed) || (a.w_packed && ks == 1 && (a.K >> 6) == 56 && a.N % 16 == 0 && a.N / 16 <= n_cu && !t.no_xs),
          "launch_gemv: the batched residual epilogue exists for the x-stationary form only (packed W, K = 3584, N / 16 <= CUs, no split-K)");
  if (a.x_packed) {
    g.nb = a.b > 16 ? 2 : 1;
    if (g.wf == WF_X12) g.wf = WF_16;
    OM_NEED(!(a.mx_scale && (a.norm_w || a.epi == EPI_RESID)), "launch_gemv: the batched norm-in-GEMV / residual forms read 16-bit weights only (no MXFP4 instantiation)");
    OM_NEED(OMCHAT_EXPERIMENTS || !(a.norm_w || a.epi == EPI_RESID), "launch_gemv: the batched norm-in-GEMV / residual forms need a -DOMCHAT_EXPERIMENTS=1 build");
    if (plan_xs(g, a, ks, t, n_cu)) return g;
    OM_NEED(!a.norm_w, "launch_gemv: packed-x RMSNorm form: gate|up shape outside the x-stationary launch (N / 32 >= 4 CUs)");
    g.family = GF_PK; g.wpack = a.w_packed != 0; g.ntile = 2; g.waves = 8; g.unroll = 4;
    if (a.epi == EPI_PARTIAL) {
      const int cps = cdiv(a.K >> 6, ks);
      if ((t.shard & 2) && cps <= 32) { g.ntile = 1; g.unroll = cps <= 8 ? 1 : 2; }
      else if (a.K / ks >= 1536) { g.ntile = 4; g.waves = 4; g.unroll = 2; }
    } else if (a.epi == EPI_NONE && a.N >= 32768) { g.ntile = 4; g.waves = 4; }
    g.gx = cdiv(cdiv(a.N, 16), g.ntile); g.gy = ks; g.block = 64 * g.waves;
    return g;
  }
  if (a.x12_top) {
    const bool ok = dtype == OMCHAT_BF16 && a.b == 1 && !a.w_packed && ks == 1 && a.K >= 512 && a.K % 512 == 0 &&
                    a.ldw == a.K / 2 * 3 && a.x12_cnt && a.x12_patch && !a.w_scale && !a.mx_scale && !mfma;
    const bool norm = ok && a.norm_w && (a.epi == EPI_SWIGLU || a.epi == EPI_NONE) && a.K <= RW_MAXC * 512;
    const bool longk = ok && !a.norm_w && a.epi == EPI_RESID && !a.out_f32 && a.K > RW_MAXC * 512 && a.K <= 32768;
    OM_NEED(norm || longk, "launch_gemv: bf16x12 weights: bf16, b == 1, K % 512 == 0, and norm_w with EPI_SWIGLU / EPI_NONE (K <= 4096) or EPI_RESID on 4096 < K <= 32768");
    if (longk) plan_longk(g, a, t, n_cu);
    else { g.rr = rows_per_wave(a, WF_X12, t, n_cu); plan_rows_norm(g, a, t, n_cu); }
    return g;
  }
  if (a.b == 1 && a.epi == EPI_RESID && ks == 1 && !a.out_f32 && a.K > RW_MAXC * 512 && a.K % 8 == 0 && a.K <= 32768 && (!mfma || a.mx_scale)) {
    plan_longk(g, a, t, n_cu);
    return g;
  }
  const bool rows_ok = a.b == 1 && cdiv(cdiv(a.K, 512), ks) <= RW_MAXC;
  OM_NEED(!a.norm_w || (rows_ok && ks == 1 && !mfma && (a.epi == EPI_NONE || a.epi == EPI_SWIGLU)),
          "launch_gemv: the in-register RMSNorm needs the whole-row batch-1 form without split-K (K <= 4096), epilogue NONE / SWIGLU");
  OM_NEED(!(a.w_scale || a.mx_scale) || rows_ok, "launch_gemv: fp8 / MXFP4 weights need b == 1 and <= 8 chunks of 512 per K slice");
  if (rows_ok && (a.w_scale || a.mx_scale || !mfma)) {
    g.rr = rows_per_wave(a, g.wf, t, n_cu);
    if (a.norm_w) plan_rows_norm(g, a, t, n_cu);
    else plan_rows(g, a, ks, t, n_cu);
    return g;
  }
  g.family = GF_MFMA; g.nb = a.b > 16 ? 2 : 1; g.waves = 8; g.unroll = 4;
  g.ntile = a.epi == EPI_SWIGLU || (a.epi == EPI_NONE && (g.nb == 2 || a.N >= 16384)) ? 2 : 1;
  if (g.nb == 1 && a.epi == EPI_PARTIAL && a.K / 64 / ks <= 32) { g.waves = 4; g.unroll = 8; }
  if (g.nb == 1 && a.epi == EPI_NONE) g.unroll = 8;
  g.gx = cdiv(a.N, 16 * g.ntile); g.gy = ks; g.block = 64 * g.waves;
  return g;
}
#undef OM_NEED

int gemv_split_k(int b, int K, int H, bool packed, bool down, const GemvTuning& t) {
  if (b == 1) { const int nch = cdiv(K, 512); return nch >= 16 ? std::min(DEC_KS_MAX, nch) : std::max(1, std::min(3, nch)); }
  if (!down && packed && K == 3584) return 2;
  if ((t.shard & 2) && K / 64 <= 64) return std::max(1, std::min(DEC_KS_MAX, (K / 64) / 16));
  return std::max(1, std::min(DEC_KS_MAX, std::min(K / 64, (down ? 3 : 1) * cdiv(512, cdiv(H, 16)))));
}

namespace {
template <auto KERNEL, typename... A>
int launch_k(const GemvPlan& g, hipStream_t s, const A&... args) {
  hipLaunchKernelGGL(KERNEL, dim3(g.gx, g.gy), dim3(g.block), (size_t)g.lds, s, args...);
  return 0;
}
template <auto KERNEL, typename... A>
int launch_k_lds64(const GemvPlan& g, hipStream_t s, const A&... args) {
  static PerDeviceOnce set;
  if (set.first()) OM_HIP(hipFuncSetAttribute((const void*)KERNEL, hipFuncAttributeMaxDynamicSharedMemorySize, 64 * 1024));
  return launch_k<KERNEL>(g, s, args...);
}
template <int... V, typename F>
int with_int(int v, F&& f) {
  int rc = -1;
  (void)((v == V ? (rc = f(std::integral_constant<int, V>{}), true) : false) || ...);
  return rc;
}
#define IV(c) decltype(c)::value
constexpr bool rows_rr(int epi, int rr, bool q) {
  return epi == EPI_NONE ? rr == 1 || rr == (q ? 8 : 4) : epi == EPI_RESID ? rr == 1 || rr == 4 : epi == EPI_SWIGLU ? rr == 4 || (rr == 1 && !q) : rr == 4;
}
constexpr bool norm_rr(int epi, int rr, bool q) { return epi == EPI_NONE ? rr == 2 || rr == 4 : q ? rr == 1 || rr == 2 || rr == 4 : rr <= 3; }

template <typename T>
int gemv_launch(const GemvPlan& g, const GemvP& p, hipStream_t s) {
  switch (g.family) {
    case GF_MFMA:
#define OM_MFMA(NT_, EPI_, WV_, UN_, NB_)                                                                  \
  if (g.ntile == NT_ && g.epi == EPI_ && g.waves == WV_ && g.unroll == UN_ && g.nb == NB_)                 \
    return launch_k<gemv_kernel<T, NT_, EPI_, WV_, UN_, false, NB_>>(g, s, p)
      OM_MFMA(1, EPI_PARTIAL, 8, 4, 2); OM_MFMA(2, EPI_SWIGLU, 8, 4, 2); OM_MFMA(1, EPI_RESID, 8, 4, 2); OM_MFMA(2, EPI_NONE, 8, 4, 2);
      OM_MFMA(1, EPI_PARTIAL, 4, 8, 1); OM_MFMA(1, EPI_PARTIAL, 8, 4, 1); OM_MFMA(2, EPI_SWIGLU, 8, 4, 1); OM_MFMA(1, EPI_RESID, 8, 4, 1);
      OM_MFMA(2, EPI_NONE, 8, 8, 1); OM_MFMA(1, EPI_NONE, 8, 8, 1);
#undef OM_MFMA
      return -1;
    case GF_PK:
#define OM_PK(NT_, EPI_, WV_, UN_)                                                                         \
  if (g.ntile == NT_ && g.epi == EPI_ && g.waves == WV_ && g.unroll == UN_)                                \
    return with_int<1, 2>(g.nb, [&](auto NB) {                                                             \
      if (g.wf == WF_MX4) return launch_k<gemv_pk_mx4_kernel<T, NT_, EPI_, WV_, UN_, IV(NB)>>(g, s, p);      \
      if (g.wpack) return launch_k<gemv_pk_kernel<T, NT_, EPI_, WV_, UN_, IV(NB), true>>(g, s, p);           \
      return launch_k<gemv_pk_kernel<T, NT_, EPI_, WV_, UN_, IV(NB), false>>(g, s, p);                       \
    })
      OM_PK(2, EPI_SWIGLU, 8, 4); OM_PK(1, EPI_PARTIAL, 8, 1); OM_PK(1, EPI_PARTIAL, 8, 2); OM_PK(4, EPI_PARTIAL, 4, 2); OM_PK(2, EPI_PARTIAL, 8, 4);
      OM_PK(4, EPI_NONE, 4, 4); OM_PK(2, EPI_NONE, 8, 4);
#undef OM_PK
      return -1;
    case GF_XS:
      return with_int<1, 2>(g.nb, [&](auto NB) {
#if OMCHAT_EXPERIMENTS
        if (g.epi == EPI_RESID) return launch_k<gemv_xs_kernel<T, EPI_RESID, IV(NB), 7>>(g, s, p);
        if (g.norm) return launch_k<gemv_xs_kernel<T, EPI_SWIGLU, IV(NB), 7, true>>(g, s, p);
#endif
        return with_int<EPI_SWIGLU, EPI_NONE>(g.epi, [&](auto EPI) {
          if (g.wf == WF_MX4) return launch_k<gemv_xs_mx4_kernel<T, IV(EPI), IV(NB), 7>>(g, s, p);
          return launch_k<gemv_xs_kernel<T, IV(EPI), IV(NB), 7>>(g, s, p);
        });
      });
    case GF_XS_SPLIT:
      return with_int<1, 2>(g.nb, [&](auto NB) {
        if (g.wf == WF_MX4) return launch_k<gemv_xs_split_mx4_kernel<T, IV(NB)>>(g, s, p, g.n5);
        return launch_k<gemv_xs_split_kernel<T, IV(NB)>>(g, s, p, g.n5);
      });
    case GF_ROWS:
      return with_int<EPI_NONE, EPI_RESID, EPI_SWIGLU, EPI_PARTIAL>(g.epi, [&](auto EPI) {
        return with_int<1, 4, 8>(g.rr, [&](auto RR) {
          auto wf = [&](auto WAVES) {
            if (rows_rr(IV(EPI), IV(RR), true)) {
              if (g.wf == WF_MX4) return launch_k<gemv_rows_mx4_kernel<T, IV(EPI), IV(RR), IV(WAVES)>>(g, s, p);
              if (g.wf == WF_E4M3) return launch_k<gemv_rows_kernel<T, IV(EPI), IV(RR), IV(WAVES), true>>(g, s, p);
            }
            if constexpr (IV(RR) != 8) if (rows_rr(IV(EPI), IV(RR), false) && g.wf == WF_16) return launch_k<gemv_rows_kernel<T, IV(EPI), IV(RR), IV(WAVES), false>>(g, s, p);
            return -1;
          };
          if constexpr (IV(EPI) == EPI_RESID && IV(RR) == 1) if (g.waves == 7) return wf(std::integral_constant<int, 7>{});
          return wf(std::integral_constant<int, 4>{});
        });
      });
    case GF_ROWS_NORM:
      return with_int<EPI_SWIGLU, EPI_NONE>(g.epi, [&](auto EPI) {
        return with_int<1, 2, 3, 4, 5, 6, 7, 8>(g.nch, [&](auto NCH) {
          if (g.wf == WF_X12) {
            constexpr int RR = IV(EPI) == EPI_SWIGLU ? 1 : 4;
            if constexpr (std::is_same<T, bf16>::value) if (g.rr == RR) return launch_k<gemv_rows_norm_x12_kernel<bf16, IV(EPI), RR, IV(NCH)>>(g, s, p);
            return -1;
          }
          if constexpr (IV(EPI) == EPI_NONE && IV(NCH) >= 4) if (g.waves == 9 && g.rr == 1) {
            if (g.wf == WF_MX4) return launch_k<gemv_rows_norm_mx4_kernel<T, IV(EPI), 1, IV(NCH), 9>>(g, s, p);
            return g.wf == WF_E4M3 ? launch_k<gemv_rows_norm_kernel<T, IV(EPI), 1, IV(NCH), true, 9>>(g, s, p) : launch_k<gemv_rows_norm_kernel<T, IV(EPI), 1, IV(NCH), false, 9>>(g, s, p);
          }
          return with_int<1, 2, 3, 4>(g.rr, [&](auto RR) {
            if constexpr (IV(RR) != 3) if (norm_rr(IV(EPI), IV(RR), true)) {
              if (g.wf == WF_MX4) return launch_k<gemv_rows_norm_mx4_kernel<T, IV(EPI), IV(RR), IV(NCH)>>(g, s, p);
              if (g.wf == WF_E4M3) return launch_k<gemv_rows_norm_kernel<T, IV(EPI), IV(RR), IV(NCH), true>>(g, s, p);
            }
            if (norm_rr(IV(EPI), IV(RR), false) && g.wf == WF_16) return launch_k<gemv_rows_norm_kernel<T, IV(EPI), IV(RR), IV(NCH), false>>(g, s, p);
            return -1;
          });
        });
      });
    case GF_ROWS_NORM_LOOP:
      return with_int<EPI_SWIGLU, EPI_NONE>(g.epi, [&](auto EPI) {
        return with_int<4, 5, 6, 7, 8>(g.nch, [&](auto NCH) {
          if (g.wf == WF_MX4) return launch_k<gemv_rows_norm_loop_mx4_kernel<T, IV(EPI), IV(NCH)>>(g, s, p, g.per_wg, g.skew);
          return g.wf == WF_E4M3 ? launch_k<gemv_rows_norm_loop_kernel<T, IV(EPI), IV(NCH), true>>(g, s, p, g.per_wg, g.skew) : launch_k<gemv_rows_norm_loop_kernel<T, IV(EPI), IV(NCH), false>>(g, s, p, g.per_wg, g.skew);
        });
      });
    case GF_ROWS_LONGK:
      if (g.wf == WF_X12) {
        if constexpr (std::is_same<T, bf16>::value) return launch_k_lds64<gemv_rows_longk_x12_kernel<T>>(g, s, p, g.rows_per_wg);
        return -1;
      }
      if (g.wf == WF_MX4) return launch_k_lds64<gemv_rows_longk_mx4_kernel<T>>(g, s, p, g.rows_per_wg);
      return g.wf == WF_E4M3 ? launch_k_lds64<gemv_rows_longk_kernel<T, true>>(g, s, p, g.rows_per_wg) : launch_k_lds64<gemv_rows_longk_kernel<T, false>>(g, s, p, g.rows_per_wg);
#if OMCHAT_EXPERIMENTS
    case GF_ROWS_NORM_DYN:
      return with_int<EPI_SWIGLU, EPI_NONE>(g.epi, [&](auto EPI) {
        return with_int<4, 5, 6, 7, 8>(g.nch, [&](auto NCH) {
          if (g.wf == WF_MX4) return launch_k<gemv_rows_norm_dyn_mx4_kernel<T, IV(EPI), IV(NCH)>>(g, s, p);
          return g.wf == WF_E4M3 ? launch_k<gemv_rows_norm_dyn_kernel<T, IV(EPI), IV(NCH), true>>(g, s, p) : launch_k<gemv_rows_norm_dyn_kernel<T, IV(EPI), IV(NCH), false>>(g, s, p);
        });
      });
    case GF_ROWS_LONGK_DIRECT:
      if (g.wf == WF_MX4) return launch_k<gemv_rows_longk_direct_mx4_kernel<T>>(g, s, p);
      return g.wf == WF_E4M3 ? launch_k<gemv_rows_longk_direct_kernel<T, true>>(g, s, p) : launch_k<gemv_rows_longk_direct_kernel<T, false>>(g, s, p);
#endif
  }
  return -1;
}
}

const GemvTuning& gemv_tuning() { return g_tune; }
void gemv_set_force_mfma(int v) { g_tune.force_mfma = v; }
int gemv_get_force_mfma() { return g_tune.force_mfma; }
void gemv_set_no_xs(int v) { g_tune.no_xs = v; }
void gemv_set_shard_shapes(int v) { g_tune.shard = v; }
int gemv_get_shard_shapes() { return g_tune.shard; }
void gemv_set_norm_loop(int v) { g_tune.norm_loop = v; }
void gemv_set_gu_rr(int v) { if (v >= 16) g_tune.gu_rr8 = v / 16; else g_tune.gu_rr = v; }
void gemv_set_dyn(int v) { g_tune.dyn = v; }
void gemv_set_longk_direct(int v) { g_tune.longk_direct = v; }
void gemv_set_skew(int v) { g_tune.skew = (unsigned)v; }
void gemv_set_rows_balance(int v) { g_tune.rows_balance = v; }
int gemv_x12_default_forms() {
  return ((g_tune.norm_loop & 1) == 0 && g_tune.gu_rr == 1 && g_tune.skew == 0u ? 1 : 0) | (g_tune.longk_direct == 0 ? 2 : 0) | ((g_tune.norm_loop & 8) == 0 ? 4 : 0);
}

namespace {
template <typename T>
__global__ __launch_bounds__(256) void quant_fp8_rows_kernel(const T* __restrict__ W, int ldw, int N, int K, unsigned char* __restrict__ W8, int ldq,
                                                             float* __restrict__ scale) {
  const int lane = threadIdx.x & 63, n = blockIdx.x * 4 + (threadIdx.x >> 6);
  if (n >= N) return;
  const T* w = W + (size_t)n * ldw;
  float m = 0.f;
  for (int k = lane * 8; k < K; k += 512) {
    const typename V8<T>::type v = ld8<T>(w + k);
#pragma unroll
    for (int j = 0; j < 8; ++j) m = fmaxf(m, fabsf(tof(v[j])));
  }
#pragma unroll
  for (int o = 32; o > 0; o >>= 1) m = fmaxf(m, __shfl_xor(m, o, 64));
  const float sc = m > 0.f ? m / 448.0f : 1.0f;
  if (lane == 0) scale[n] = sc;
  for (int k = lane * 8; k < K; k += 512) {
    const typename V8<T>::type v = ld8<T>(w + k);
    float f[8];
#pragma unroll
    for (int j = 0; j < 8; ++j) f[j] = tof(v[j]) / sc;
    int lo = 0, hi = 0;
    lo = __builtin_amdgcn_cvt_pk_fp8_f32(f[0], f[1], lo, false);
    lo = __builtin_amdgcn_cvt_pk_fp8_f32(f[2], f[3], lo, true);
    hi = __builtin_amdgcn_cvt_pk_fp8_f32(f[4], f[5], hi, false);
    hi = __builtin_amdgcn_cvt_pk_fp8_f32(f[6], f[7], hi, true);
    rw_u32x2 o2 = {(unsigned)lo, (unsigned)hi};
    *reinterpret_cast<rw_u32x2*>(W8 + (size_t)n * ldq + k) = o2;
  }
}
}

int launch_quant_fp8_rows(int dtype, const void* W, int ldw, int N, int K, void* W8, int ld8, float* scale, hipStream_t s) {
  OM_CHECK(K % 8 == 0 && ldw % 8 == 0 && ld8 % 8 == 0, "K, ldw, ld8 must be multiples of 8");
  if (dtype == OMCHAT_F16) hipLaunchKernelGGL(quant_fp8_rows_kernel<f16>, dim3(cdiv(N, 4)), dim3(256), 0, s, (const f16*)W, ldw, N, K, (unsigned char*)W8, ld8, scale);
  else if (dtype == OMCHAT_BF16) hipLaunchKernelGGL(quant_fp8_rows_kernel<bf16>, dim3(cdiv(N, 4)), dim3(256), 0, s, (const bf16*)W, ldw, N, K, (unsigned char*)W8, ld8, scale);
  else { omchat_set_error("launch_quant_fp8_rows: bad dtype"); return 1; }
  OM_LAUNCH_CHECK();
  return 0;
}

namespace {
template <typename T>
__global__ __launch_bounds__(256) void quant_mxfp4_rows_kernel(const T* __restrict__ W, int ldw, int N, int K, unsigned char* __restrict__ W4, int ld4,
                                                               unsigned char* __restrict__ S) {
  const int lane = threadIdx.x & 63, n = blockIdx.x * 4 + (threadIdx.x >> 6);
  if (n >= N) return;
  const T* w = W + (size_t)n * ldw;
  for (int k = lane * 8; k < K; k += 512) {
    const typename V8<T>::type v = ld8<T>(w + k);
// ... 230 lines not shown
```

### omchat_amd/csrc/kernels.h

```cpp
#pragma once
#ifndef OMCHAT_EXPERIMENTS
#define OMCHAT_EXPERIMENTS 0
#endif
#include "common.h"
#if OMCHAT_EXPERIMENTS
#include <hip/hip_ext.h>
extern int g_launch_any_order;
#undef hipLaunchKernelGGL
#define hipLaunchKernelGGL(kernelName, numBlocks, numThreads, memPerBlock, streamId, ...)                                                      \
  do {                                                                                                                                         \
    if (g_launch_any_order)                                                                                                                    \
      hipExtLaunchKernelGGL((kernelName), dim3(numBlocks), dim3(numThreads), (memPerBlock), (streamId), nullptr, nullptr, hipExtAnyOrderLaunch, \
                            __VA_ARGS__);                                                                                                      \
    else                                                                                                                                       \
      hipLaunchKernelGGLInternal((kernelName), numBlocks, numThreads, memPerBlock, streamId, __VA_ARGS__);                                     \
  } while (0)
#endif

enum {
  EPI_NONE = 0,
  EPI_GELU = 1,
  EPI_LS_RESID = 2,
  EPI_RESID = 3,
  EPI_SWIGLU = 4,
// ... 5 lines not shown
};
struct GemmArgs {
  const void* A; int lda;
  const void* W; int ldw;
  void* C; int ldc;
  int M, N, K;
  const void* bias;
  const void* ls;
  const void* resid;
  int ldr;
  int epi;
  int force_tile;
  void* sk_ws; size_t sk_ws_bytes;
  int stream_k;
  int f8;
  const float* a_scale; const float* w_scale;
  const float* row_scale = nullptr;
  const float* rs_stats = nullptr; int rs_ld = 0, rs_nslots = 0, rs_dim = 0; float rs_eps = 0.f;
  float* stats = nullptr; int stats_ld = 0; int* stats_nslots = nullptr;
  const int* lse_labels = nullptr; float* lse_tgt = nullptr;
};
int launch_gemm(int dtype, const GemmArgs& a, hipStream_t stream);
int launch_stats_finish(const float* stats, int ld, int slot0, int nslots, int ngroups, int rows, int dim, float eps, float* out, hipStream_t s);
int launch_row_sumsq(int dtype, const void* x, int ldx, int rows, int H, float* stats, hipStream_t s);
size_t gemm_sk_ws_bytes();
void gemm_set_skew(int v);
void gemm_set_persist(int v);
void gemm_set_wide_store(int v);
void gemm_set_skip_dead(int v);

struct GemvArgs {
  const void* X; int ldx;
  const void* W; int ldw;
  void* Y; int ldy;
  int b, N, K;
  const void* bias;
  const void* resid; int ldr;
  int epi;
  int out_f32;
  int ksplit;
  int force_mfma;
  const float* w_scale;
  int x_packed;
  int w_packed;
  int y_packed;
  const void* norm_w; float norm_eps;
  void* dyn_ctr = nullptr;
  void* y_pack = nullptr;
  unsigned long long* dbg = nullptr;
  const unsigned char* mx_scale = nullptr;
  const unsigned char* x12_top = nullptr;
  const unsigned char* x12_cnt = nullptr;
  const unsigned* x12_patch = nullptr;
};
int launch_encode_bf16x12(const void* W, int ldw, int N, int K, void* coded, unsigned char* top, unsigned char* cnt, unsigned* patch, int* over,
                          hipStream_t stream);
int launch_pack_x(int dtype, const void* X, int ldx, int b, int K, void* out, hipStream_t s);
int launch_pack_w(int dtype, const void* W, int ldw, int N, int K, void* out, hipStream_t s);
int launch_pack_w4(const void* W4, const unsigned char* S, int N, int K, void* W4P, unsigned char* SP, hipStream_t s);
int launch_gemv(int dtype, const GemvArgs& a, hipStream_t stream);
struct GemvTuning {
  int force_mfma = 0, no_xs = 0, shard = 15, norm_loop = 0, gu_rr = 1, gu_rr8 = 1, dyn = 0, longk_direct = 0, rows_balance = 1;
  unsigned skew = 0;
};
const GemvTuning& gemv_tuning();
enum GemvFamily { GF_MFMA = 0, GF_PK, GF_XS, GF_XS_SPLIT, GF_ROWS, GF_ROWS_NORM, GF_ROWS_NORM_LOOP, GF_ROWS_LONGK, GF_ROWS_NORM_DYN, GF_ROWS_LONGK_DIRECT };
constexpr int WF_16 = 0, WF_E4M3 = 1, WF_MX4 = 2, WF_X12 = 3;
struct GemvPlan {
  const char* refusal;
  int family, wf, wpack, epi, ntile, waves, unroll, nb, rr, nch, norm;
  int gx, gy, block, lds;
  int per_wg; unsigned skew;
  int rows_per_wg;
  int n5;
  int xskew;
};
GemvPlan gemv_plan(int dtype, const GemvArgs& a, const GemvTuning& t, int n_cu);
constexpr int DEC_KS_MAX = 8;
int gemv_split_k(int b, int K, int H, bool packed, bool down, const GemvTuning& t);
int launch_gemv_wait(int dtype, const GemvArgs& a, const unsigned* flags, unsigned epoch, int nflags, unsigned* err, int mode, hipStream_t s);
int launch_quant_fp8_rows(int dtype, const void* W, int ldw, int N, int K, void* W8, int ld8, float* scale, hipStream_t stream);
int launch_quant_mxfp4_rows(int dtype, const void* W, int ldw, int N, int K, void* W4, int ld4, unsigned char* S, hipStream_t stream);
void gemv_set_force_mfma(int v);
int gemv_get_force_mfma();
void gemm_set_autotune(int v);
int gemm_tune_load(const char* path);
int gemm_tune_dump(const char* path);
long gemm_tune_runs();
void model_set_ar_min_rows(int v);
void model_set_tp_f32(int v);
void model_set_pack_replica(int v);
void model_set_norm_in_gemv(int v);
void model_set_vit_fused(int v);
void model_set_tp_sp(int v);
int launch_fold_cols(int dtype, const void* W, const void* n, void* out, int rows, int cols, hipStream_t s);

int launch_layernorm(int dtype, const void* x, int ldx, const void* w, const void* b, void* y, int ldy, int rows, int H, float eps, hipStream_t stream);
int launch_rmsnorm(int dtype, const void* x, int ldx, const void* w, void* y, int ldy, int rows, int H, float eps, hipStream_t s, int pack_nb = 0);
int launch_rmsnorm_q8(int dtype, const void* x, int ldx, const void* w, void* y8, int ldy, float* scale, int rows, int H, float eps, hipStream_t s);
int launch_quant_rows_q8(int dtype, const void* x, int ldx, void* y8, int ldy, float* scale, int rows, int H, hipStream_t s);
int launch_resid_rmsnorm(int dtype, void* x, int ldx, const float* part, int ks, const void* w, void* xn, int ldn, int rows, int H, float eps,
                         hipStream_t s, int pack_nb = 0);
int launch_resid16_norm(int dtype, void* x, int ldx, const void* y, int ldy, const void* w, const void* b, void* xn, int ldn, int rows, int H, float eps,
                        hipStream_t s);
int launch_vit_qknorm(int dtype, void* qkv, int ld, const void* wq, const void* wk, int rows, int C, int C_total,
                      float eps, float q_scale, const float* sumsq_in, hipStream_t s, int only_k = 0);
int launch_vit_qk_sumsq(int dtype, const void* qkv, int ld, int rows, int C, float* sumsq_out, hipStream_t s);
int launch_vit_knorm_slots(int dtype, void* k, int ld, const void* wk, int rows, int C, int C_total, float eps, const float* stats, int stats_ld, int nslots,
                           float* sumsq_q, hipStream_t s);
struct AttnArgs {
  const void* Q; int64_t q_sb, q_sh, q_sr;
  const void* K; int64_t k_sb, k_sh, k_sr;
  const void* V; int64_t v_sb, v_sh, v_sr;
  void* O; int64_t o_sb, o_sh, o_sr;
  int batch, q_heads, kv_heads;
  int Sq, Skv;
  const int* kv_len;
  const int* kv_start;
  int causal;
  int q_pos0;
  float scale;
  int head_dim;
  const float* qn_sumsq = nullptr; int qn_stride = 0, qn_dim = 0; const void* qn_w = nullptr; float qn_eps = 0.f, qn_scale = 1.f;
};
int launch_attn_prefill(int dtype, const AttnArgs& a, hipStream_t s);
int launch_attn_uniform_rows(int dtype, const AttnArgs& a, hipStream_t s);
void attn_set_v2(int v);
void model_set_fuse_peer_norm(int v);
void attn_set_tpw(int v);
void attn_set_klds(int v);
void attn_set_dma(int v);
void attn_set_dma_slots(int v);
void attn_set_dma_rot(int v);
void attn_set_hsplit(int v);
void attn_set_mha_xcd(int v);
void attn_set_kg(int v);
void attn_set_peel(int v);
void attn_set_kv8_tpw(int v);
void attn_set_kv8_fuse(int v);
void model_set_extend_attn(int v);
void model_set_x12_roles(int v);
void model_set_suffix_attn(int v);
int gemv_x12_default_forms();
bool attn_decode_kv8_fuses_rope(int batch, int kv_heads, int L, bool masked);
void attn_set_merge_mid_min(int v);
void attn_set_merge_dg(int v);
void gemv_set_norm_loop(int v);
void gemv_set_dyn(int v);
void gemv_set_skew(int v);
void gemv_set_rows_balance(int v);
void gemv_set_no_xs(int v);
void gemv_set_shard_shapes(int v);
void gemv_set_gu_rr(int v);
void gemv_set_longk_direct(int v);
void norm_set_wave(int v);
void model_set_ao_oproj(int v);
int gemv_get_shard_shapes();

struct AttnOperands {
  const void* Q; int64_t q_sb, q_sh;
  const void* K; int64_t k_sb, k_sh, k_sr;
  const void* V; int64_t v_sb, v_sh, v_sr;
  void* O; int64_t o_sb, o_sh;
  int q_heads, kv_heads;
  float scale;
  float* ws; size_t ws_bytes;
  const float* rope; int rope_max;
  const void* k_new; const void* v_new; int64_t new_sb;
  int o_pack_nb;
};

struct AttnDecodeArgs : AttnOperands {
  int batch;
  int L;
  const int* kv_len;
  const int* pos;
  const float* k_scale; const float* v_scale; int64_t scale_sb, scale_sh;
  void* k16_w = nullptr; void* v16_w = nullptr;
  const unsigned char* key_mask; int64_t mask_sb;
  unsigned* done_flags = nullptr; unsigned done_epoch = 0; int done_mode = 0;
  unsigned long long* done_dbg = nullptr;
};
int launch_kv_quant(int dtype, const void* kc, const void* vc, void* k8, void* v8, float* ks, float* vs, int b, int kv_heads, int64_t c_sb, int64_t c_sh,
                    int64_t s_sb, int64_t s_sh, const int* pos_lo, int pos0, const int* len, int max_rows, hipStream_t s);
size_t attn_decode_ws_bytes(int batch, int q_heads, int max_len);
int launch_attn_decode(int dtype, const AttnDecodeArgs& a, hipStream_t s);
int launch_attn_merge(int dtype, const float* ws, int nsplit, int q_heads, int rows, const int* kv_len, int L, float scale, void* O, int split_keys,
                      hipStream_t s);

enum AttnBlockMode { ATTN_VERIFY = 0, ATTN_EXTEND, ATTN_SHARED, ATTN_SUFFIX };
struct AttnBlockArgs : AttnOperands {
  int mode;
  int G, N, S, P, L;
  const int* kv_len;
};
// ... 207 lines not shown
```

### omchat_amd/csrc/model.hip

```cpp
#include "ctx.h"
#include <limits.h>
#include <math.h>
#include <string.h>
#include <algorithm>
#include <functional>
#include <string>
#include <unordered_map>
#include <vector>

static thread_local std::string g_err;
void omchat_set_error(const std::string& s) { g_err = s; }
extern "C" const char* omchat_last_error(void) { return g_err.c_str(); }
extern "C" const char* omchat_version(void) { return "omchat_hip 0.1 (gfx950)"; }

namespace {

__global__ void cast_from_f32_f16(const float* s, f16* d, int64_t n) {
  for (int64_t i = (int64_t)blockIdx.x * blockDim.x + threadIdx.x; i < n; i += (int64_t)gridDim.x * blockDim.x) d[i] = (f16)s[i];
}
__global__ void cast_from_f32_bf16(const float* s, bf16* d, int64_t n) {
  for (int64_t i = (int64_t)blockIdx.x * blockDim.x + threadIdx.x; i < n; i += (int64_t)gridDim.x * blockDim.x) d[i] = (bf16)s[i];
}
__global__ void add_positions_kernel(int* pos, int b, int d) {
  const int i = threadIdx.x;
// ... 845 lines not shown
  OM_HIP(hipMemcpyAsync(P.dola_hid, xf, (size_t)b * H * 2, hipMemcpyDeviceToDevice, s));
  TRY(launch_rmsnorm(ctx->dt, P.dola_hid, H, ctx->t_norm, P.dola_hid, H, P.dola.norm ? n : b, H, c.t_eps, s));
  TRY(lm_head_rows(ctx, P.dola_hid, n, P.dola_logits, s, ctx->lm_w(OMCHAT_WFMT_16)));
  if (logits) OM_HIP(hipMemcpyAsync(logits, P.dola_logits, (size_t)b * c.t_vocab * 4, hipMemcpyDeviceToDevice, s));
  P.dola_fresh = true;
  return 0;
}
static void* dola_slot(omchat_ctx* ctx, int j) { return (char*)ctx->pick.dola_hid + (size_t)(1 + j) * ctx->pick.dola.b * ctx->c.t_hidden * 2; }

static int build_replica(omchat_ctx* ctx, int fmt) {
  omchat_ctx::WTable& T = ctx->wt[fmt];
  if (T.state == omchat_ctx::W_BUILT) return 0;
  const bool f8 = fmt == OMCHAT_WFMT_E4M3, mx = fmt == OMCHAT_WFMT_MXFP4, mxp = fmt == OMCHAT_WFMT_MXFP4_PACKED, p16 = fmt == OMCHAT_WFMT_16_PACKED;
  if (f8 || mx) OM_CHECK(omchat_weights_missing(ctx) == 0, "load the weights before quantising them");
  if (mx) OM_CHECK(ctx->c.t_hidden % 32 == 0 && ctx->t_qdim % 32 == 0 && ctx->c.t_mlp % 32 == 0,
                   "MXFP4 decode: every streamed K (hidden_size, heads x 128, intermediate_size) must be a multiple of 32");
  if (mxp) TRY(build_replica(ctx, OMCHAT_WFMT_MXFP4));
  const std::vector<omchat_ctx::WRef>& src = ctx->wt[mxp ? OMCHAT_WFMT_MXFP4 : OMCHAT_WFMT_16].e;
  if (T.e.empty()) {
    std::vector<omchat_ctx::WRef> fresh(src.size());
    std::vector<void**> slots;
    std::vector<size_t> sizes;
    for (size_t j = 0; j < fresh.size(); ++j) {
      const size_t N = entry_shape(ctx, j).N, K = entry_shape(ctx, j).K;
      omchat_ctx::WRef& r = fresh[j];
      r.ldw = (int)(mx || mxp ? K / 2 : K);
      r.packed = p16 || mxp;
      slots.push_back(&r.W); sizes.push_back(p16 ? N * K * 2 : f8 ? N * K : N * (K / 2));
      if (f8) { slots.push_back((void**)&r.w_scale); sizes.push_back(N * 4); }
      if (mx || mxp) { slots.push_back((void**)&r.mx_scale); sizes.push_back(N * (K / 32)); }
    }
    if (ctx->alloc_group(slots, sizes)) {
      if (p16) { T.state = omchat_ctx::W_UNAVAILABLE; return 0; }
      if (mxp) omchat_set_error("omchat_enable_mxfp4_decode: the packed MXFP4 replica of mode 2 does not fit in device memory (hipMalloc failed)");
      return 2;
    }
    T.e.swap(fresh);
  }
  for (size_t j = 0; j < T.e.size(); ++j) {
    const int N = entry_shape(ctx, j).N, K = entry_shape(ctx, j).K;
    const omchat_ctx::WRef& w = src[j]; const omchat_ctx::WRef& r = T.e[j];
    if (f8) TRY(launch_quant_fp8_rows(ctx->dt, w.W, K, N, K, r.W, K, r.w_scale, nullptr));
    else if (mx) TRY(launch_quant_mxfp4_rows(ctx->dt, w.W, K, N, K, r.W, K / 2, r.mx_scale, nullptr));
    else if (mxp) TRY(launch_pack_w4(w.W, w.mx_scale, N, K, r.W, r.mx_scale, nullptr));
    else TRY(launch_pack_w(ctx->dt, w.W, K, N, K, r.W, nullptr));
  }
  OM_HIP(hipDeviceSynchronize());
  T.state = omchat_ctx::W_BUILT;
  return 0;
}

int g_x12_roles = 7;
void model_set_x12_roles(int v) { g_x12_roles = v & 7; }

static int x12_step_mask(const omchat_ctx* ctx, int rows, int fmt) {
  if (rows != 1 || fmt != OMCHAT_WFMT_16 || ctx->dt != OMCHAT_BF16 || ctx->tp_size != 1) return 0;
  return g_x12_roles & gemv_x12_default_forms();
}

static int build_x12(omchat_ctx* ctx, int role) {
  omchat_ctx::X12Table& T = ctx->x12[role];
  if (T.state == omchat_ctx::W_BUILT || T.state == omchat_ctx::W_UNAVAILABLE) return 0;
  const omchat_config& c = ctx->c;
  const int H = c.t_hidden, It = c.t_mlp, L = c.t_layers;
  const bool lm = role == omchat_ctx::X12_LM, down = role == omchat_ctx::X12_DOWN;
  const size_t N = lm ? c.t_vocab : down ? H : 2 * (size_t)It, K = down ? It : H, n = lm ? 1 : L;
  const bool k_ok = K % 512 == 0 && (down ? (K > 4096 && K <= 32768) : K <= 4096);
  if (!k_ok || omchat_weights_missing(ctx) != 0) { if (!k_ok) T.state = omchat_ctx::W_UNAVAILABLE; return 0; }
  if (T.e.empty()) {
    std::vector<omchat_ctx::X12Ref> fresh(n);
    std::vector<void**> slots;
    std::vector<size_t> sizes;
    for (auto& r : fresh) {
      slots.push_back(&r.W); sizes.push_back(N * (K / 2 * 3));
      slots.push_back((void**)&r.top); sizes.push_back(N);
      slots.push_back((void**)&r.cnt); sizes.push_back(N);
      slots.push_back((void**)&r.patch); sizes.push_back(N * 32 * 4);
    }
    int* over = nullptr;
    if (!ctx->x12_over) { slots.push_back((void**)&over); sizes.push_back((size_t)std::max(L, 1) * 4); }
    if (ctx->alloc_group(slots, sizes)) { T.state = omchat_ctx::W_UNAVAILABLE; return 0; }
    if (over) ctx->x12_over = over;
    T.e.swap(fresh);
  }
  OM_HIP(hipDeviceSynchronize());
  OM_HIP(hipMemset(ctx->x12_over, 0, n * 4));
  for (size_t j = 0; j < n; ++j) {
    const void* W = lm ? ctx->lm_w(OMCHAT_WFMT_16).W : ctx->layer_w(OMCHAT_WFMT_16, (int)j)[down ? omchat_ctx::P_DOWN : omchat_ctx::P_GU].W;
    const omchat_ctx::X12Ref& r = T.e[j];
    TRY(launch_encode_bf16x12(W, (int)K, (int)N, (int)K, r.W, r.top, r.cnt, r.patch, ctx->x12_over + j, nullptr));
  }
  OM_HIP(hipDeviceSynchronize());
  std::vector<int> over(n);
  OM_HIP(hipMemcpy(over.data(), ctx->x12_over, n * 4, hipMemcpyDeviceToHost));
  bool moved = false;
  for (size_t j = 0; j < n; ++j) { moved = moved || (T.state == omchat_ctx::W_STALE && T.e[j].ok != !over[j]); T.e[j].ok = !over[j]; }
  if (moved) drop_decode_graphs(ctx);
  T.state = omchat_ctx::W_BUILT;
  return 0;
}

extern "C" int omchat_enable_fp8_decode(omchat_ctx* ctx, int on) {
  OM_CHECK(ctx, "null context");
  OM_CHECK(ctx->c.t_layers > 0, "context has no decoder");
  if (!on) { ctx->fp8_decode = false; return 0; }
  OM_CHECK(!ctx->mxfp4_mode, "MXFP4 decode is on: one weight format per step (omchat_enable_mxfp4_decode(ctx, 0) first)");
  OM_CHECK(!on || !ctx->pick.dola_on(), "fp8 decode: layer-contrastive decoding is on, and its head pass is 16-bit only (omchat_set_dola with b = 0 first)");
  TRY(build_replica(ctx, OMCHAT_WFMT_E4M3));
  ctx->fp8_decode = true;
  return 0;
}

extern "C" int omchat_enable_mxfp4_decode(omchat_ctx* ctx, int mode) {
  OM_CHECK(ctx, "null context");
  OM_CHECK(ctx->c.t_layers > 0, "context has no decoder");
  OM_CHECK(mode >= 0 && mode <= 2, "mode: 0 = off, 1 = batch-1 steps, 2 = steps of up to 32 rows as well");
  if (!mode) { ctx->mxfp4_mode = 0; return 0; }
  OM_CHECK(!ctx->fp8_decode, "fp8 decode is on: one weight format per step (omchat_enable_fp8_decode(ctx, 0) first)");
  OM_CHECK(!mode || !ctx->pick.dola_on(), "MXFP4 decode: layer-contrastive decoding is on, and its head pass is 16-bit only (omchat_set_dola with b = 0 first)");
  OM_CHECK(ctx->tp_size == 1, "MXFP4 decode under tensor parallelism is not implemented");
  if (mode == 2) {
    const omchat_config& c = ctx->c;
    OM_CHECK(c.t_hidden % 64 == 0 && ctx->t_qdim % 64 == 0 && c.t_mlp % 64 == 0,
             "MXFP4 decode mode 2: the packed path needs hidden_size, heads x 128 and intermediate_size each a multiple of 64");
    OM_CHECK(ctx->t_qkvdim % 16 == 0 && c.t_hidden % 16 == 0 && c.t_vocab % 16 == 0,
             "MXFP4 decode mode 2: the packed path needs the qkv width, hidden_size and vocab_size each a multiple of 16");
  }
  TRY(build_replica(ctx, mode == 2 ? OMCHAT_WFMT_MXFP4_PACKED : OMCHAT_WFMT_MXFP4));
  ctx->mxfp4_mode = mode;
  return 0;
}

extern "C" int omchat_enable_fp8_kv(omchat_ctx* ctx, int on) {
  OM_CHECK(ctx, "null context");
  const omchat_config& c = ctx->c;
  OM_CHECK(c.t_layers > 0, "context has no decoder");
  ctx->kv8_valid = false;
  if (!on) { ctx->fp8_kv = false; return 0; }
  if (!ctx->k8cache) {
    const size_t bytes = (size_t)c.t_layers * ctx->cache_layer_stride();
    const size_t sc = (size_t)c.t_layers * ctx->scale_layer_stride() * 4;
// ... 357 lines not shown
    for (int r0 = 0; r0 < b; r0 += 32) {
      const int R = std::min(32, b - r0);
      const GemvArgs g = gemv_args((const char*)X + (size_t)r0 * ldx * 2, ldx, W, K, (char*)Y + (size_t)r0 * ldy * 2, ldy, R, N, bias,
                                   resid ? (const char*)resid + (size_t)r0 * H * 2 : nullptr, epi, 0, ypk);
      TRY(launch_gemv(ctx->dt, g, s));
    }
    return 0;
  };
  auto gemv_partial = [&](const void* X, int ldx, const WRef& W, int K, int ks) -> int {
    OM_CHECK(b <= 32, "split-K decode path handles b <= 32");
    const GemvArgs g = gemv_args(X, ldx, W, K, ctx->tw_part, H, b, H, nullptr, nullptr, EPI_PARTIAL, ks, false);
    TRY(launch_gemv(ctx->dt, g, s));
    return 0;
  };
  const bool fused = b <= 32;
  const int ks_o = gemv_split_k(b, qd, H, wpk || mpk, false, gemv_tuning()), ks_d = gemv_split_k(b, It, H, wpk || mpk, true, gemv_tuning());
  const bool tp1_like = ctx->tp_size == 1 || (OMCHAT_EXPERIMENTS && g_shard_as_tp1 && ctx->hook == omchat_allreduce_noop);
  const bool n2 = (g_norm_in_gemv & 1) && fused && b == 1 && tp1_like && qd <= 4096 && H <= 4096 && !gemv_get_force_mfma();
  const bool n1 = n2 && (g_norm_in_gemv & 2) && It <= 32768 && It % 8 == 0;
  const bool nb2 = OMCHAT_EXPERIMENTS && (g_norm_in_gemv & 4) && fused && wpk && ctx->tp_size == 1 && !wq && (qd >> 6) == 56 && (H >> 6) == 56 && qd % 64 == 0 &&
                   H / 16 <= device_cus() && (2 * It) / 32 >= 4 * device_cus();
  const int x12m = n1 ? x12_step_mask(ctx, b, fmt) : 0;
  auto x12_of = [&](int role, size_t j) -> const omchat_ctx::X12Ref* {
    const omchat_ctx::X12Table& T = ctx->x12[role];
    return ((x12m >> role) & 1) && T.state == omchat_ctx::W_BUILT && T.e[j].ok ? &T.e[j] : nullptr;
  };
  if (fused && !n1) TRY(launch_rmsnorm(ctx->dt, x, H, ctx->dl[0].ln1, ctx->tw_xn, H, b, H, c.t_eps, s, pk));
#if OMCHAT_EXPERIMENTS
  if ((g_ao_oproj & 16) && ctx->dbg_stamps) OM_HIP(hipMemsetAsync(ctx->dbg_stamps, 0, (size_t)c.t_layers * 256, s));
#endif
  for (int i = 0; i < c.t_layers; ++i) {
    auto& L = ctx->dl[i];
    const WRef* W = ctx->layer_w(fmt, i);
    const WRef* W16 = ctx->layer_w(OMCHAT_WFMT_16, i);
    char* kc = (char*)ctx->kcache + (size_t)i * ctx->cache_layer_stride() * 2;
    char* vc = (char*)ctx->vcache + (size_t)i * ctx->cache_layer_stride() * 2;
    if (!fused) TRY(launch_rmsnorm(ctx->dt, x, H, L.ln1, ctx->tw_xn, H, b, H, c.t_eps, s));
    if (g_decode_layer && !dola && n1 && exact_len && !masked && !wq && !(ctx->fp8_kv && ctx->kv8_valid) && ctx->dl_ws) {
      DecodeLayerArgs d{L.ln1, L.ln2, W16[QKV].W, L.bqkv, W16[O].W, W16[GU].W, W16[DOWN].W, kc, vc, ctx->cache_sh(), x, H, qd, ctx->t_kvdim, It, c.t_heads, c.t_kv_heads, Lmax,
                        ctx->rope, c.max_seq, c.t_eps, omchat_ctx::T_ATTN_SCALE, ctx->dl_ws, ++ctx->fd_epoch, ctx->fd_err, 2000};
      if (decode_layer_ok(d)) {
        const bool mark_l = allow_prof && i == c.t_layers / 2;
        if (mark_l) ctx->prof_mark(OMCHAT_PROF_DECODE_GATEUP, s);
        TRY(launch_decode_layer(ctx->dt, d, s));
        if (mark_l) ctx->prof_mark(OMCHAT_PROF_DECODE_GATEUP, s);
        ++ctx->n_layer_launches;
        continue;
      }
      --ctx->fd_epoch;
    }
    if (n1) {
      GemvArgs g = gemv_args(x, H, W[QKV], H, ctx->tw_qkv, qkvd, 1, qkvd, L.bqkv, nullptr, EPI_NONE, 0, false);
      g.norm_w = L.ln1; g.norm_eps = c.t_eps;
      if (OMCHAT_EXPERIMENTS && (g_ao_oproj & 16) && ctx->dbg_stamps) g.dbg = ctx->dbg_stamps + (size_t)i * 32;
      TRY(launch_gemv(ctx->dt, g, s));
    } else {
      TRY(gemv(ctx->tw_xn, H, W[QKV], H, ctx->tw_qkv, qkvd, qkvd, L.bqkv, nullptr, EPI_NONE));
    }
    AttnDecodeArgs a{};
    ctx->bind_attn(a, i, true);
    a.ws = ctx->tw_attn_ws; a.ws_bytes = ctx->tw_attn_ws_bytes;
    a.o_pack_nb = fused ? pk : 0;
    a.batch = b; a.L = Lmax; a.kv_len = exact_len ? nullptr : ctx->d_len; a.pos = ctx->d_pos;
    if (masked) { a.key_mask = ctx->d_mask; a.mask_sb = ctx->mask_sb; }
    if (ctx->fp8_kv && ctx->kv8_valid) {
      const size_t off = (size_t)i * ctx->cache_layer_stride(), so = (size_t)i * ctx->scale_layer_stride();
      RopeArgs r{ctx->tw_qkv, qkvd, b, 1, c.t_heads, c.t_kv_heads, ctx->d_pos, 0, ctx->rope, c.max_seq, kc, vc, ctx->cache_sb(), ctx->cache_sh()};
      r.k8 = (char*)ctx->k8cache + off; r.v8 = (char*)ctx->v8cache + off; r.ks = ctx->ks8 + so; r.vs = ctx->vs8 + so;
      r.s_sb = (int64_t)c.t_kv_heads * c.max_seq; r.s_sh = c.max_seq;
      if (masked) r.slot0 = Lmax - 1;
      else if (exact_len) { r.pos = nullptr; r.pos0 = Lmax - 1; }
      if (attn_decode_kv8_fuses_rope(b, c.t_kv_heads, Lmax, masked)) { a.k16_w = kc; a.v16_w = vc; a.pos = nullptr; }
      else {
        TRY(launch_rope_kv(ctx->dt, r, s));
        a.rope = nullptr; a.pos = nullptr; a.k_new = nullptr; a.v_new = nullptr;
      }
      a.K = (char*)ctx->k8cache + off; a.V = (char*)ctx->v8cache + off;
      a.k_scale = ctx->ks8 + so; a.v_scale = ctx->vs8 + so; a.scale_sb = (int64_t)c.t_kv_heads * c.max_seq; a.scale_sh = c.max_seq;
    }
    bool ao_oproj = false;
    const bool fuse_ao = g_fuse_attn_oproj && !dola && n2 && exact_len && !wq && a.rope && ctx->fd_ws && attn_oproj_fused_ok(a, H, qd);
    if (vL < 0 && ctx->group.on()) {
      const GroupState& G = ctx->group;
      AttnBlockArgs sa{};
      static_cast<AttnOperands&>(sa) = a;
      sa.ws = (float*)G.ws.p; sa.ws_bytes = G.ws.cap;
      sa.mode = ATTN_SHARED; sa.G = G.b; sa.N = G.N; sa.P = G.P; sa.L = Lmax; sa.kv_len = ctx->d_len;
      TRY(launch_attn_block(ctx->dt, sa, s));
    } else if (vL >= 0) {
      AttnBlockArgs va{};
      static_cast<AttnOperands&>(va) = a;
      va.mode = ATTN_VERIFY; va.S = b; va.L = vL;
      TRY(launch_attn_block(ctx->dt, va, s));
    } else if (fuse_ao) {
      FusedDecodeArgs fa{W16[O].W, qd, x, H, qd, ctx->fd_ws, ++ctx->fd_epoch, ctx->fd_err, 2000};
      TRY(launch_attn_oproj_fused(ctx->dt, a, fa, s));
      ++ctx->n_fused_launches;
    } else {
#if OMCHAT_EXPERIMENTS
      ao_oproj = (g_ao_oproj & 1) && n2 && !wq && !masked && ctx->fd_ws && Lmax <= 4096 && H == 3584 && qd == 3584 && c.t_heads <= 64 && !ctx->graph_on;
      if (ao_oproj) { a.done_flags = (unsigned*)ctx->fd_ws; a.done_epoch = ++ctx->fd_epoch; a.done_mode = g_ao_oproj; }
      if ((g_ao_oproj & 16) && n2 && ctx->dbg_stamps) a.done_dbg = ctx->dbg_stamps + (size_t)i * 32;
#endif
      TRY(launch_attn_decode(ctx->dt, a, s));
    }
    if (fuse_ao) {
    } else if (ao_oproj) {
      GemvArgs g = gemv_args(ctx->tw_ao, qd, W16[O], qd, x, H, 1, H, nullptr, x, EPI_RESID, 0, false);
      if ((g_ao_oproj & 16) && ctx->dbg_stamps) g.dbg = ctx->dbg_stamps + (size_t)i * 32;
      TRY(launch_gemv_wait(ctx->dt, g, (const unsigned*)ctx->fd_ws, ctx->fd_epoch, c.t_heads, ctx->fd_err, g_ao_oproj, s));
    } else if (n2 && OMCHAT_EXPERIMENTS && (g_ao_oproj & 16) && ctx->dbg_stamps && !wq) {
      GemvArgs g = gemv_args(ctx->tw_ao, qd, W16[O], qd, x, H, 1, H, nullptr, x, EPI_RESID, 0, false);
      g.dbg = ctx->dbg_stamps + (size_t)i * 32;
      TRY(launch_gemv(ctx->dt, g, s));
    } else if (n2) {
      TRY(gemv(ctx->tw_ao, qd, W[O], qd, x, H, H, nullptr, x, EPI_RESID));
    } else if (nb2) {
      GemvArgs g = gemv_args(ctx->tw_ao, qd, W[O], qd, x, H, b, H, nullptr, x, EPI_RESID, 0, false);
      g.y_pack = ctx->tw_xn;
      TRY(launch_gemv(ctx->dt, g, s));
    } else if (fused) {
      TRY(gemv_partial(ctx->tw_ao, qd, W[O], qd, ks_o));
      TRY(ctx->reduce_resid_rmsnorm(x, H, ctx->tw_part, ks_o, L.ln2, ctx->tw_xn, H, b, H, c.t_eps, pk, s));
    } else if (ctx->tp_size == 1) {
      TRY(gemv(ctx->tw_ao, qd, W[O], qd, x, H, H, nullptr, x, EPI_RESID));
    } else {
      TRY(gemv(ctx->tw_ao, qd, W[O], qd, y, H, H, nullptr, lead ? x : nullptr, lead ? EPI_RESID : EPI_NONE));
      TRY(ctx->allreduce(y, (size_t)b * H, s));
      std::swap(x, y);
    }
    if (!fused) TRY(launch_rmsnorm(ctx->dt, x, H, L.ln2, ctx->tw_xn, H, b, H, c.t_eps, s));
    const bool mark = allow_prof && i == c.t_layers / 2;
    if (mark) ctx->prof_mark(OMCHAT_PROF_DECODE_GATEUP, s);
    if (n2) {
      GemvArgs g = gemv_args(x, H, W[GU], H, ctx->tw_act, It, 1, 2 * It, nullptr, nullptr, EPI_SWIGLU, 0, false);
      g.norm_w = L.ln2; g.norm_eps = c.t_eps;
      if (const auto* r = x12_of(omchat_ctx::X12_GU, i)) { use_weight_x12(g, *r, H); ++ctx->x12_launches[omchat_ctx::X12_GU]; }
      if (ctx->dyn_ctr && !ctx->graph_on) g.dyn_ctr = ctx->dyn_ctr + (size_t)i * 65 * 64;
      if (OMCHAT_EXPERIMENTS && (g_ao_oproj & 16) && ctx->dbg_stamps) g.dbg = ctx->dbg_stamps + (size_t)i * 32;
      TRY(launch_gemv(ctx->dt, g, s));
    } else if (nb2) {
      GemvArgs g = gemv_args(ctx->tw_xn, H, W[GU], H, ctx->tw_act, It, b, 2 * It, nullptr, nullptr, EPI_SWIGLU, 0, true);
      g.norm_w = L.ln2; g.norm_eps = c.t_eps;
      TRY(launch_gemv(ctx->dt, g, s));
    } else {
      TRY(gemv(ctx->tw_xn, H, W[GU], H, ctx->tw_act, It, 2 * It, nullptr, nullptr, EPI_SWIGLU, true));
    }
    if (mark) ctx->prof_mark(OMCHAT_PROF_DECODE_GATEUP, s);
    if (n1 && OMCHAT_EXPERIMENTS && (g_ao_oproj & 16) && ctx->dbg_stamps && !wq) {
      GemvArgs g = gemv_args(ctx->tw_act, It, W16[DOWN], It, x, H, 1, H, nullptr, x, EPI_RESID, 0, false);
      g.dbg = ctx->dbg_stamps + (size_t)i * 32;
      TRY(launch_gemv(ctx->dt, g, s));
    } else if (n1 && x12_of(omchat_ctx::X12_DOWN, i)) {
      GemvArgs g = gemv_args(ctx->tw_act, It, W[DOWN], It, x, H, 1, H, nullptr, x, EPI_RESID, 0, false);
      use_weight_x12(g, *x12_of(omchat_ctx::X12_DOWN, i), It);
      ++ctx->x12_launches[omchat_ctx::X12_DOWN];
      TRY(launch_gemv(ctx->dt, g, s));
    } else if (n1) {
      TRY(gemv(ctx->tw_act, It, W[DOWN], It, x, H, H, nullptr, x, EPI_RESID));
    } else if (fused) {
      TRY(gemv_partial(ctx->tw_act, It, W[DOWN], It, ks_d));
      const void* nw = i + 1 < c.t_layers ? ctx->dl[i + 1].ln1 : ctx->t_norm;
      TRY(ctx->reduce_resid_rmsnorm(x, H, ctx->tw_part, ks_d, nw, ctx->tw_xn, H, b, H, c.t_eps, pk, s));
    } else if (ctx->tp_size == 1) {
      TRY(gemv(ctx->tw_act, It, W[DOWN], It, x, H, H, nullptr, x, EPI_RESID));
    } else {
      TRY(gemv(ctx->tw_act, It, W[DOWN], It, y, H, H, nullptr, lead ? x : nullptr, lead ? EPI_RESID : EPI_NONE));
// ... 6 lines not shown
  float* lg = logits ? logits : ctx->tw_logits;
  int pick_b = b;
  if (dola) {
    TRY(dola_head(ctx, x, logits, s));
    lg = ctx->pick.dola_logits; pick_b = D.rows();
  } else if (n1) {
    GemvArgs g{x, H, nullptr, 0, lg, c.t_vocab, 1, c.t_vocab, H, nullptr, nullptr, 0, EPI_NONE, 1};
    use_weight(g, ctx->lm_w(fmt));
    if (const auto* r = x12_of(omchat_ctx::X12_LM, 0)) { use_weight_x12(g, *r, H); ++ctx->x12_launches[omchat_ctx::X12_LM]; }
    g.norm_w = ctx->t_norm; g.norm_eps = c.t_eps;
    TRY(launch_gemv(ctx->dt, g, s));
  } else {
    TRY(lm_head_rows(ctx, ctx->tw_xn, b, lg, s, ctx->lm_w(fmt), fused && pk));
  }
  if (vL >= 0) TRY(pick_verify(ctx, lg, b, tokens, next_tokens, s, vsample));
  else if (next_tokens) TRY(pick_run(ctx, lg, pick_b, next_tokens, s, true, tokens));
  else {
    hipLaunchKernelGGL(advance_lens_kernel, dim3(1), dim3(64 > b ? 64 : b), 0, s, ctx->d_pos, ctx->d_len, b);
    TRY(pick_feed(ctx, tokens, b, s));
  }
  OM_LAUNCH_CHECK();
  return 0;
}

static void destroy_graph(omchat_ctx::DecodeGraph& g) {
  if (g.exec) (void)hipGraphExecDestroy(g.exec);
  if (g.graph) (void)hipGraphDestroy(g.graph);
  g = omchat_ctx::DecodeGraph{};
}

void drop_decode_graphs(omchat_ctx* ctx) {
  for (auto& kv : ctx->graphs) destroy_graph(kv.second);
  ctx->graphs.clear();
}


extern "C" int omchat_enable_decode_graph(omchat_ctx* ctx, int on) {
  OM_CHECK(ctx, "null ctx");
  OM_CHECK(ctx->c.t_layers > 0, "context has no decoder");
  if (on && !ctx->graph_stream) {
    OM_HIP(hipStreamCreateWithFlags(&ctx->graph_stream, hipStreamNonBlocking));
    OM_HIP(hipEventCreateWithFlags(&ctx->graph_ev_in, hipEventDisableTiming));
    OM_HIP(hipEventCreateWithFlags(&ctx->graph_ev_out, hipEventDisableTiming));
    TRY(ctx->alloc((void**)&ctx->d_tok_in, (size_t)ctx->c.max_batch * 4));
    TRY(ctx->alloc((void**)&ctx->d_tok_out, (size_t)ctx->c.max_batch * 4));
  }
  ctx->graph_on = on != 0;
  return 0;
}

extern "C" int omchat_bf16x12_stats(omchat_ctx* ctx, int* roles, long* launches, int* coded) {
  OM_CHECK(ctx, "null context");
  if (roles) *roles = g_x12_roles;
  for (int r = 0; r < omchat_ctx::X12_ROLES; ++r) {
    if (launches) launches[r] = ctx->x12_launches[r];
    int n = 0;
    if (ctx->x12[r].state == omchat_ctx::W_BUILT) for (const auto& e : ctx->x12[r].e) n += e.ok ? 1 : 0;
    if (coded) coded[r] = n;
  }
  return 0;
}

extern "C" int omchat_decode_graph_stats(omchat_ctx* ctx, long* steps, long* replays, long* captures) {
  OM_CHECK(ctx, "null ctx");
  if (steps) *steps = ctx->graph_steps;
  if (replays) *replays = ctx->graph_replays;
  if (captures) *captures = ctx->graph_captures;
  return 0;
}

extern "C" int omchat_decode_step(omchat_ctx* ctx, const int32_t* tokens, int b, float* logits, int32_t* next_tokens, void* stream) {
  OM_CHECK(ctx && tokens, "null argument");
  const omchat_config& c = ctx->c;
  OM_CHECK(c.t_layers > 0, "context has no decoder");
  OM_CHECK(b >= 1 && b <= c.max_batch, "batch exceeds max_batch");
  OM_CHECK(mx4_rows_ok(ctx, b), MX4_ROWS_MSG);
  if (const char* why = pick_rows_refusal(ctx, b)) OM_CHECK(false, why);
  if (ctx->pick.dola_on())
    if (const char* why = dola_state_refusal(ctx)) OM_CHECK(false, why);
  int Lmax = 0;
  OM_CHECK(!ctx->left_padded, "per-sequence decode after a left-padded prefill: use omchat_decode_step_masked (the reference positions such a "
                              "batch with sum(mask) - 1 and a per-row key mask, omchat_arch.py:61-70; DESIGN.md section 7)");
  OM_CHECK(ctx->dec_mode != 2, "omchat_decode_step after omchat_decode_step_masked on the same prefill: the two place the cache rows differently");
  bool same_len = true;
  int Lmin = c.max_seq;
  for (int i = 0; i < b; ++i) {
    OM_CHECK(ctx->h_len[i] >= 1, "decode before prefill");
    Lmax = std::max(Lmax, ctx->h_len[i] + 1);
    Lmin = std::min(Lmin, ctx->h_len[i]);
    same_len = same_len && ctx->h_len[i] == ctx->h_len[0];
  }
  OM_CHECK(Lmax <= c.max_seq, "KV cache full (max_seq)");
  hipStream_t s = (hipStream_t)stream;
  GroupState& G = ctx->group;
  const bool grp = G.on();
  if (grp) {
    OM_CHECK(b == G.b * G.N && Lmin >= G.P, "a sampled group shares its prompt: a step takes all its b * N rows, none shorter than the prompt (omchat_group_begin with b = 0 first)");
    OM_CHECK(ctx->tp_size == 1 && !(ctx->fp8_kv && ctx->kv8_valid), "shared-prompt mode: one GPU, 16-bit KV cache");
    Lmax = std::min(c.max_seq, G.P + (Lmax - G.P + 255) / 256 * 256);
    const size_t need = attn_shared_ws_bytes(G.b, G.N, c.t_heads, c.t_kv_heads, G.P, Lmax);
    if (need > G.ws.cap) TRY(ctx->grow(G.ws, attn_shared_ws_bytes(G.b, G.N, c.t_heads, c.t_kv_heads, G.P, std::min(c.max_seq, Lmax + 768))));
  }
  TRY(step_weights_ready(ctx, b));
  TRY(pick_admit(ctx, next_tokens != nullptr, true));
  ctx->graph_steps++;
  const bool graph = ctx->graph_on && ctx->tp_size == 1 && b <= 32 && !(ctx->prof_on && ctx->graph_steps % 8 == 0);
  if (!graph) {
    TRY(decode_body(ctx, tokens, b, Lmax, logits, next_tokens, s, true, same_len && !grp));
  } else {
    const int fmt = step_format(ctx, b);
    omchat_ctx::DecodeGraph& g = ctx->graphs[b * 8 + (is_mxfp4(fmt) ? 4 : 0) + (fmt == OMCHAT_WFMT_E4M3 ? 2 : 0) + ((ctx->fp8_kv && ctx->kv8_valid) ? 1 : 0) +
// ... 310 lines not shown
```

### omchat_amd/engine.py

```python
import ctypes as C
import numpy as np

from . import _lib
from ._lib import OmchatConfig, check, ptr, cur_stream
from .config import OmChatConfig


def _torch():
    import torch
    return torch


GROUP_SHARE_P_MIN = 2048


def group_share_refusal(fp8_kv, tp_size, q_heads, kv_heads, N):
    if fp8_kv:
        return "the e4m3 KV cache"
    if tp_size != 1:
        return "tensor parallelism"
    if not 2 <= N <= 16 or N * (q_heads // max(1, kv_heads)) > 128:
        return "N outside 2 <= N <= 16 and N * (q heads per kv head) <= 128"
    return None

# ... 110 lines not shown
        return t

    def encode_images_dp(self, tower, pixels, select_layer=-1):
        torch = _torch()
        n = pixels.shape[0]
        out = torch.zeros(n, self.ntok, self.cfg.text["hidden_size"], dtype=self.torch_dtype, device=self.device)
        lo, hi = self.tp_rank * n // self.tp_size, (self.tp_rank + 1) * n // self.tp_size
        if hi > lo:
            out[lo:hi] = tower.encode_images(pixels[lo:hi], select_layer)
        return self.allreduce(out)

    def comm_stats(self):
        a, b = C.c_long(0), C.c_long(0)
        check(self.lib.omchat_ctx_comm_stats(self.h, C.byref(a), C.byref(b)))
        rs, ag = C.c_long(0), C.c_long(0)
        check(self.lib.omchat_ctx_sp_stats(self.h, C.byref(rs), C.byref(ag)))
        return dict(peer_allreduces=a.value, rccl_allreduces=b.value, sp_reduce_scatters=rs.value, sp_all_gathers=ag.value)

    def enable_fp8_decode(self, on=True):
        check(self.lib.omchat_enable_fp8_decode(self.h, int(on)))
        self._fp8_decode = bool(on)

    def enable_mxfp4_decode(self, on=True, batched=False):
        check(self.lib.omchat_enable_mxfp4_decode(self.h, (2 if batched else 1) if on else 0))
        self._mxfp4_decode = bool(on)
        self._mxfp4_batched = bool(on) and bool(batched)

    def enable_fp8_kv(self, on=True):
        check(self.lib.omchat_enable_fp8_kv(self.h, int(on)))
        self._fp8_kv = bool(on)
        self._prefix = None

    def masked_decode_supported(self):
        return self.tp_size == 1

    def enable_fp8_prefill(self, on=True):
        check(self.lib.omchat_enable_fp8_prefill(self.h, int(on)))
        self._fp8_prefill = bool(on)
        self._prefix = None

    def enable_decode_graph(self, on=True):
        check(self.lib.omchat_enable_decode_graph(self.h, int(on)))

    def decode_graph_stats(self):
        st, rp, cp = C.c_long(0), C.c_long(0), C.c_long(0)
        check(self.lib.omchat_decode_graph_stats(self.h, C.byref(st), C.byref(rp), C.byref(cp)))
        return dict(steps=st.value, replays=rp.value, captures=cp.value)

    def bf16x12_stats(self):
        roles, launches, coded = C.c_int(0), (C.c_long * 3)(), (C.c_int * 3)()
        check(self.lib.omchat_bf16x12_stats(self.h, C.byref(roles), launches, coded))
        return dict(roles=roles.value, launches=list(launches), coded=list(coded))

    def prof_enable(self, on=True):
        check(self.lib.omchat_prof_enable(self.h, int(on)))

    def prof_read(self, cat, reset=True):
        ms, n = C.c_double(0), C.c_long(0)
        check(self.lib.omchat_prof_read(self.h, cat, C.byref(ms), C.byref(n), int(reset)))
        return ms.value, n.value

    def device_bytes(self):
        return int(self.lib.omchat_device_bytes(self.h))

    def _px(self, pixels):
        torch = _torch()
        if pixels.dim() != 4 or pixels.shape[1] != 3:
            raise ValueError(f"wrong pixel_values size: {tuple(pixels.shape)}")
        s = self.cfg.vision["image_size"]
        if pixels.shape[2] != s or pixels.shape[3] != s:
            raise ValueError(f"expected {s}x{s} tiles, got {tuple(pixels.shape[2:])}")
        return pixels.to(device=self.device, dtype=self.torch_dtype).contiguous()

    def vit_forward(self, pixels, select_layer=-1, select_feature="patch"):
        torch = _torch()
        if select_feature not in ("patch", "cls_patch"):
            raise ValueError(f"Unexpected select feature: {select_feature}")
        px = self._px(pixels)
        n = px.shape[0]
        keep = select_feature == "cls_patch"
        out = torch.empty(n, self.ntok + (1 if keep else 0), self.cfg.vision["hidden_size"], dtype=self.torch_dtype, device=self.device)
        check(self.lib.omchat_vit_forward(self.h, ptr(px), n, select_layer, int(keep), ptr(out), cur_stream()))
        return out

    def projector_forward(self, x):
        torch = _torch()
        x = x.to(device=self.device, dtype=self.torch_dtype).contiguous()
        rows = x.numel() // x.shape[-1]
        out = torch.empty(*x.shape[:-1], self.cfg.text["hidden_size"], dtype=self.torch_dtype, device=self.device)
        check(self.lib.omchat_projector_forward(self.h, ptr(x), rows, ptr(out), cur_stream()))
        return out

    def encode_images(self, pixels, select_layer=-1):
        torch = _torch()
        px = self._px(pixels)
        n = px.shape[0]
        out = torch.empty(n, self.ntok, self.cfg.text["hidden_size"], dtype=self.torch_dtype, device=self.device)
        check(self.lib.omchat_encode_images(self.h, ptr(px), n, select_layer, ptr(out), cur_stream()))
        self._enc_st["calls"] += 1; self._enc_st["tiles"] += n
        return out

    def encode_stats(self, reset=False):
        out = dict(self._enc_st)
        if reset:
            self._enc_st = dict(calls=0, tiles=0)
        return out
# ... 469 lines not shown
```

Baseline: 391.3.

## Extend bf16x12 compressed weight GEMV to QKV and O projections in decode

Adds two new bf16x12 roles (QKV and O projection) so that single-row bf16 decode at TP=1 reads 12-bit coded weights for the attention projections as well as for the MLP and LM head. It adds dedicated kernels: a 9-wave fused-norm rows kernel for QKV and a 7-wave residual rows kernel for o_proj, both using a grouped dot helper. The goal is to cut the weight bytes read per decode step. The cost is extra encode time, extra memory for the coded tables, and patch/decode work inside the kernel. The metric is dominated by prefill and TTFT, so the change may matter little there.

```diff
diff --git a/include/omchat_hip.h b/include/omchat_hip.h
--- a/include/omchat_hip.h
+++ b/include/omchat_hip.h
@@ -134,6 +134,7 @@
 int omchat_enable_decode_graph(omchat_ctx* ctx, int on);
 int omchat_decode_graph_stats(omchat_ctx* ctx, long* steps, long* replays, long* captures);
 int omchat_bf16x12_stats(omchat_ctx* ctx, int* roles, long* launches, int* coded);
+int omchat_bf16x12_short_stats(omchat_ctx* ctx, int* roles, long* launches, int* coded);
 
 int omchat_enable_fp8_decode(omchat_ctx* ctx, int on);
 
@@ -212,6 +213,8 @@
 int omchat_op_encode_bf16x12(const void* W, int N, int K, void* coded, void* top, void* cnt, void* patch, void* over, void* stream);
 int omchat_op_gemv_bf16x12(const void* X, const void* coded, const void* top, const void* cnt, const void* patch, void* Y, int N, int K,
                            const void* norm_w, float eps, const void* resid, int epi, int out_f32, void* stream);
+int omchat_op_gemv_bf16x12_short(const void* X, const void* coded, const void* top, const void* cnt, const void* patch, void* Y, int N, int K,
+                                 const void* norm_w, float eps, const void* bias, const void* resid, void* stream);
 int omchat_op_pack_w(int dtype, const void* W, int ldw, int N, int K, void* out, void* stream);
 int omchat_op_pack_w4(const void* W4, const void* S, int N, int K, void* W4P, void* SP, void* stream);
 int omchat_op_gemv_prepacked(int dtype, const void* XP, const void* WP, const void* SP, void* Y, int ldy, int b, int N, int K, const void* bias,
diff --git a/omchat_amd/_lib.py b/omchat_amd/_lib.py
--- a/omchat_amd/_lib.py
+++ b/omchat_amd/_lib.py
@@ -115,6 +115,7 @@
     "omchat_enable_fp8_prefill": (_i, [_vp, _i]),
     "omchat_enable_decode_graph": (_i, [_vp, _i]),
     "omchat_bf16x12_stats": (_i, [_vp, C.POINTER(_i), C.POINTER(C.c_long), C.POINTER(_i)]),
+    "omchat_bf16x12_short_stats": (_i, [_vp, C.POINTER(_i), C.POINTER(C.c_long), C.POINTER(_i)]),
     "omchat_decode_graph_stats": (_i, [_vp, C.POINTER(C.c_long), C.POINTER(C.c_long), C.POINTER(C.c_long)]),
     "omchat_op_quant_fp8": (_i, [_i, _vp, _i, _i, _vp, _vp, _vp]),
     "omchat_op_gemv_fp8": (_i, [_i, _vp, _vp, _vp, _vp, _i, _i, _vp, _vp, _i, _i, _i, _vp]),
@@ -129,6 +130,7 @@
     "omchat_op_gemv_prepacked": (_i, [_i, _vp, _vp, _vp, _vp, _i, _i, _i, _i, _vp, _i, _i, _i, _i, _vp]),
     "omchat_op_encode_bf16x12": (_i, [_vp, _i, _i, _vp, _vp, _vp, _vp, _vp, _vp]),
     "omchat_op_gemv_bf16x12": (_i, [_vp, _vp, _vp, _vp, _vp, _vp, _i, _i, _vp, _f, _vp, _i, _i, _vp]),
+    "omchat_op_gemv_bf16x12_short": (_i, [_vp, _vp, _vp, _vp, _vp, _vp, _i, _i, _vp, _f, _vp, _vp, _vp]),
     "omchat_op_gemv_mxfp4_norm": (_i, [_i, _vp, _vp, _vp, _vp, _i, _i, _vp, _f, _vp, _i, _i, _vp]),
     "omchat_op_rmsnorm": (_i, [_i, _vp, _vp, _vp, _i, _i, _f, _vp]),
     "omchat_op_resid_rmsnorm": (_i, [_i, _vp, _i, _vp, _i, _vp, _vp, _i, _i, _i, _f, _i, _vp]),
diff --git a/omchat_amd/csrc/capi.hip b/omchat_amd/csrc/capi.hip
--- a/omchat_amd/csrc/capi.hip
+++ b/omchat_amd/csrc/capi.hip
@@ -97,6 +97,7 @@
   if (key == 49) { model_set_extend_attn(value); return 0; }
   if (key == 50) { model_set_x12_roles(value); return 0; }
   if (key == 51) { model_set_suffix_attn(value); return 0; }
+  if (key == 52) { model_set_x12_short(value); return 0; }
   if (key == 38) { gemv_set_gu_rr(value); return 0; }
   if (key == 39) { gemv_set_longk_direct(value); return 0; }
   if (key == 40) { norm_set_wave(value); return 0; }
@@ -170,6 +171,7 @@
   if (wf == WF_E4M3) a.w_scale = (const float*)set;
   if (wf == WF_MX4) a.mx_scale = (const unsigned char*)set;
   if (wf == WF_X12) { a.x12_top = a.x12_cnt = (const unsigned char*)set; a.x12_patch = set; }
+  a.x12_short = flags >> 7 & 1;
   const GemvPlan g = gemv_plan(dtype, a, gemv_tuning(), n_cu > 0 ? n_cu : device_cus());
   if (g.refusal) { omchat_set_error(g.refusal); return 1; }
   const int f[OMCHAT_GEMV_PLAN_INTS] = {g.family, g.wf, g.wpack, g.epi, g.ntile, g.waves, g.unroll, g.nb, g.rr, g.nch, g.norm, g.gx, g.gy, g.block, g.lds,
@@ -982,6 +984,15 @@
   g.x12_top = (const unsigned char*)top; g.x12_cnt = (const unsigned char*)cnt; g.x12_patch = (const unsigned*)patch;
   return launch_gemv(OMCHAT_BF16, g, S(stream));
 }
+extern "C" int omchat_op_gemv_bf16x12_short(const void* X, const void* coded, const void* top, const void* cnt, const void* patch, void* Y, int N, int K,
+                                            const void* norm_w, float eps, const void* bias, const void* resid, void* stream) {
+  OM_CHECK(X && coded && top && cnt && patch && Y && (norm_w || resid), "null argument");
+  GemvArgs g{X, K, coded, K / 2 * 3, Y, N, 1, N, K, bias, norm_w ? nullptr : resid, N, norm_w ? EPI_NONE : EPI_RESID, 0};
+  g.norm_w = norm_w; g.norm_eps = eps;
+  g.x12_top = (const unsigned char*)top; g.x12_cnt = (const unsigned char*)cnt; g.x12_patch = (const unsigned*)patch;
+  g.x12_short = 1;
+  return launch_gemv(OMCHAT_BF16, g, S(stream));
+}
 
 extern "C" int omchat_op_attn_prefill_d(int dtype, const void* q, const void* k, const void* v, void* out, int b, int Sq, int Skv, int Hq,
                                         int Hkv, int D, const int32_t* kv_len, int causal, int q_pos0, float scale, void* stream) {
diff --git a/omchat_amd/csrc/ctx.h b/omchat_amd/csrc/ctx.h
--- a/omchat_amd/csrc/ctx.h
+++ b/omchat_amd/csrc/ctx.h
@@ -153,12 +153,12 @@
   const WRef* layer_w(int fmt, int layer) const { return &wt[fmt].e[(size_t)layer * 4]; }
   const WRef& lm_w(int fmt) const { return wt[fmt].e.back(); }
   bool built(int fmt) const { return wt[fmt].state == W_BUILT; }
-  enum X12Role { X12_GU = 0, X12_DOWN = 1, X12_LM = 2, X12_ROLES = 3 };
+  enum X12Role { X12_GU = 0, X12_DOWN = 1, X12_LM = 2, X12_LONG_ROLES = 3, X12_QKV = 3, X12_O = 4, X12_ROLES = 5 };
   struct X12Ref { void* W = nullptr; unsigned char* top = nullptr; unsigned char* cnt = nullptr; unsigned* patch = nullptr; bool ok = false; };
   struct X12Table { std::vector<X12Ref> e; int state = W_ABSENT; };
   X12Table x12[X12_ROLES];
   int* x12_over = nullptr;
-  long x12_launches[X12_ROLES] = {0, 0, 0};
+  long x12_launches[X12_ROLES] = {0, 0, 0, 0, 0};
   bool fp8_decode = false;
   int mxfp4_mode = 0;
   void *k8cache = nullptr, *v8cache = nullptr;
diff --git a/omchat_amd/csrc/gemv.hip b/omchat_amd/csrc/gemv.hip
--- a/omchat_amd/csrc/gemv.hip
+++ b/omchat_amd/csrc/gemv.hip
@@ -726,6 +726,20 @@
   }
 }
 
+template <typename T, int GS, int NCH, int C0 = 0>
+__device__ __forceinline__ float x12_row_dots(const X12W* w, X12Row& s, const rw_u32x4* xr, int c_lo, int lane, float a) {
+  if constexpr (C0 < NCH) {
+    constexpr int G = NCH - C0 < GS ? NCH - C0 : GS;
+    rw_u32x4 wd[G];
+    x12_group<G>(wd, w + C0, s, c_lo + C0, c_lo + NCH, lane);
+#pragma unroll
+    for (int c = 0; c < G; ++c) a = rw_dot8<T>(wd[c], xr[C0 + c], a);
+    return x12_row_dots<T, GS, NCH, C0 + G>(w, s, xr, c_lo, lane, a);
+  } else {
+    return a;
+  }
+}
+
 template <typename T, int WF>
 __device__ __forceinline__ typename RwW<WF>::type rw_ldw(const GemvP& p, size_t row, int k) {
   if constexpr (WF == WF_X12) return x12_ldw(p, row, k >> 9, (k >> 3) & 63); else
@@ -779,12 +793,36 @@
   }
 }
 
+template <typename T, int R, int NCH>
+__device__ __forceinline__ void rw_rows_x12(const GemvP& p, const int (&rows)[R], int k0, int lane, const rw_u32x4 (&xr)[RW_MAXC], float (&acc)[R],
+                                            RwTail<T, R>& tail) {
+  X12W w[R][NCH];
+#pragma unroll
+  for (int r = 0; r < R; ++r)
+#pragma unroll
+    for (int c = 0; c < NCH; ++c) w[r][c] = rw_ldw<T, WF_X12>(p, (size_t)rows[r], k0 + c * 512 + lane * 8);
+  X12Row xst[R];
+#pragma unroll
+  for (int r = 0; r < R; ++r) x12_row_load(xst[r], p, (size_t)rows[r], lane);
+  rw_tail_load<T, R>(tail);
+#pragma unroll
+  for (int r = 0; r < R; ++r) {
+    x12_row_finish(xst[r]);
+    float a = x12_row_dots<T, 2, NCH>(&w[r][0], xst[r], xr, k0 >> 9, lane, 0.f);
+#pragma unroll
+    for (int o = 32; o > 0; o >>= 1) a += __shfl_xor(a, o, 64);
+    acc[r] = a;
+  }
+}
+
 template <typename T, int R, int N, int WF>
 __device__ __forceinline__ void rw_dispatch_q(int nch, const GemvP& p, const int (&rows)[R], int k0, int lane, const rw_u32x4 (&xr)[RW_MAXC],
                                               float (&acc)[R], RwTail<T, R>& tail) {
   if constexpr (N > 0) {
-    if (nch == N) rw_rows_q<T, R, N, WF>(p, rows, k0, lane, xr, acc, tail);
-    else rw_dispatch_q<T, R, N - 1, WF>(nch, p, rows, k0, lane, xr, acc, tail);
+    if (nch == N) {
+      if constexpr (WF == WF_X12) rw_rows_x12<T, R, N>(p, rows, k0, lane, xr, acc, tail);
+      else rw_rows_q<T, R, N, WF>(p, rows, k0, lane, xr, acc, tail);
+    } else rw_dispatch_q<T, R, N - 1, WF>(nch, p, rows, k0, lane, xr, acc, tail);
   }
 }
 
@@ -898,6 +936,8 @@
 __global__ __launch_bounds__(WAVES * 64) void gemv_rows_kernel(GemvP p) { gemv_rows_body<T, EPI, RR, WAVES, F8 ? WF_E4M3 : WF_16>(p); }
 template <typename T, int EPI, int RR, int WAVES>
 __global__ __launch_bounds__(WAVES * 64) void gemv_rows_mx4_kernel(GemvP p) { gemv_rows_body<T, EPI, RR, WAVES, WF_MX4>(p); }
+template <typename T>
+__global__ __launch_bounds__(448) void gemv_rows_x12_kernel(GemvP p) { gemv_rows_body<T, EPI_RESID, 1, 7, WF_X12>(p); }
 
 template <typename T, int EPI, int RR, int NCH, int F8, int WAVES>
 __device__ __forceinline__ void gemv_rows_norm_body(const GemvP& p) {
@@ -1033,7 +1073,9 @@
     for (int c = 0; c < NCH; ++c) {
       if constexpr (F8 != WF_X12) a = rw_dotw<T, F8>(w[r][c], xr[c], a);
     }
-    if constexpr (F8 == WF_X12) {
+    if constexpr (F8 == WF_X12 && WAVES == 9) {
+      a = x12_row_dots<T, 2, NCH>(&w[r][0], xst[r], xr, 0, lane, a);
+    } else if constexpr (F8 == WF_X12) {
       constexpr int G0 = NCH < 4 ? NCH : 4, G1 = NCH - G0;
       {
         rw_u32x4 wd[G0];
@@ -1078,6 +1120,8 @@
 __global__ __launch_bounds__(WAVES * 64) void gemv_rows_norm_mx4_kernel(GemvP p) { gemv_rows_norm_body<T, EPI, RR, NCH, WF_MX4, WAVES>(p); }
 template <typename T, int EPI, int RR, int NCH>
 __global__ __launch_bounds__(256) void gemv_rows_norm_x12_kernel(GemvP p) { gemv_rows_norm_body<T, EPI, RR, NCH, WF_X12, 4>(p); }
+template <typename T, int NCH>
+__global__ __launch_bounds__(576) void gemv_rows_norm_x12w9_kernel(GemvP p) { gemv_rows_norm_body<T, EPI_NONE, 1, NCH, WF_X12, 9>(p); }
 
 template <typename T, int EPI, int NCH, int F8>
 __device__ __forceinline__ void gemv_rows_norm_loop_body(const GemvP& p, int per_wg, unsigned skew) {
@@ -1725,6 +1769,15 @@
   if (a.x12_top) {
     const bool ok = dtype == OMCHAT_BF16 && a.b == 1 && !a.w_packed && ks == 1 && a.K >= 512 && a.K % 512 == 0 &&
                     a.ldw == a.K / 2 * 3 && a.x12_cnt && a.x12_patch && !a.w_scale && !a.mx_scale && !mfma;
+    if (a.x12_short) {
+      const bool qkv = ok && a.norm_w && a.epi == EPI_NONE && a.K <= RW_MAXC * 512;
+      const bool oproj = ok && !a.norm_w && a.epi == EPI_RESID && !a.out_f32 && a.K <= RW_MAXC * 512;
+      OM_NEED(qkv || oproj, "launch_gemv: bf16x12 short rows: bf16, b == 1, K % 512 == 0, K <= 4096, and norm_w with EPI_NONE (qkv) or EPI_RESID without norm_w (o_proj)");
+      g.family = qkv ? GF_ROWS_NORM : GF_ROWS; g.rr = 1; g.waves = qkv ? 9 : 7; g.block = 64 * g.waves;
+      if (qkv) g.nch = a.K / 512;
+      g.gx = cdiv(a.N, g.waves);
+      return g;
+    }
     const bool norm = ok && a.norm_w && (a.epi == EPI_SWIGLU || a.epi == EPI_NONE) && a.K <= RW_MAXC * 512;
     const bool longk = ok && !a.norm_w && a.epi == EPI_RESID && !a.out_f32 && a.K > RW_MAXC * 512 && a.K <= 32768;
     OM_NEED(norm || longk, "launch_gemv: bf16x12 weights: bf16, b == 1, K % 512 == 0, and norm_w with EPI_SWIGLU / EPI_NONE (K <= 4096) or EPI_RESID on 4096 < K <= 32768");
@@ -1827,6 +1880,10 @@
         return launch_k<gemv_xs_split_kernel<T, IV(NB)>>(g, s, p, g.n5);
       });
     case GF_ROWS:
+      if (g.wf == WF_X12) {
+        if constexpr (std::is_same<T, bf16>::value) if (g.epi == EPI_RESID && g.rr == 1 && g.waves == 7) return launch_k<gemv_rows_x12_kernel<bf16>>(g, s, p);
+        return -1;
+      }
       return with_int<EPI_NONE, EPI_RESID, EPI_SWIGLU, EPI_PARTIAL>(g.epi, [&](auto EPI) {
         return with_int<1, 4, 8>(g.rr, [&](auto RR) {
           auto wf = [&](auto WAVES) {
@@ -1845,6 +1902,7 @@
       return with_int<EPI_SWIGLU, EPI_NONE>(g.epi, [&](auto EPI) {
         return with_int<1, 2, 3, 4, 5, 6, 7, 8>(g.nch, [&](auto NCH) {
           if (g.wf == WF_X12) {
+            if constexpr (std::is_same<T, bf16>::value && IV(EPI) == EPI_NONE) if (g.waves == 9 && g.rr == 1) return launch_k<gemv_rows_norm_x12w9_kernel<bf16, IV(NCH)>>(g, s, p);
             constexpr int RR = IV(EPI) == EPI_SWIGLU ? 1 : 4;
             if constexpr (std::is_same<T, bf16>::value) if (g.rr == RR) return launch_k<gemv_rows_norm_x12_kernel<bf16, IV(EPI), RR, IV(NCH)>>(g, s, p);
             return -1;
@@ -1907,7 +1965,8 @@
 void gemv_set_skew(int v) { g_tune.skew = (unsigned)v; }
 void gemv_set_rows_balance(int v) { g_tune.rows_balance = v; }
 int gemv_x12_default_forms() {
-  return ((g_tune.norm_loop & 1) == 0 && g_tune.gu_rr == 1 && g_tune.skew == 0u ? 1 : 0) | (g_tune.longk_direct == 0 ? 2 : 0) | ((g_tune.norm_loop & 8) == 0 ? 4 : 0);
+  return ((g_tune.norm_loop & 1) == 0 && g_tune.gu_rr == 1 && g_tune.skew == 0u ? 1 : 0) | (g_tune.longk_direct == 0 ? 2 : 0) | ((g_tune.norm_loop & 8) == 0 ? 4 : 0) |
+         ((g_tune.norm_loop & 2) == 0 && g_tune.rows_balance ? 8 : 0) | (g_tune.rows_balance ? 16 : 0);
 }
 
 namespace {
diff --git a/omchat_amd/csrc/kernels.h b/omchat_amd/csrc/kernels.h
--- a/omchat_amd/csrc/kernels.h
+++ b/omchat_amd/csrc/kernels.h
@@ -81,6 +81,7 @@
   const unsigned char* x12_top = nullptr;
   const unsigned char* x12_cnt = nullptr;
   const unsigned* x12_patch = nullptr;
+  int x12_short = 0;
 };
 int launch_encode_bf16x12(const void* W, int ldw, int N, int K, void* coded, unsigned char* top, unsigned char* cnt, unsigned* patch, int* over,
                           hipStream_t stream);
@@ -170,6 +171,7 @@
 void model_set_extend_attn(int v);
 void model_set_x12_roles(int v);
 void model_set_suffix_attn(int v);
+void model_set_x12_short(int v);
 int gemv_x12_default_forms();
 bool attn_decode_kv8_fuses_rope(int batch, int kv_heads, int L, bool masked);
 void attn_set_merge_mid_min(int v);
diff --git a/omchat_amd/csrc/model.hip b/omchat_amd/csrc/model.hip
--- a/omchat_amd/csrc/model.hip
+++ b/omchat_amd/csrc/model.hip
@@ -921,10 +921,13 @@
 
 int g_x12_roles = 7;
 void model_set_x12_roles(int v) { g_x12_roles = v & 7; }
+int g_x12_short = 3;
+void model_set_x12_short(int v) { g_x12_short = v & 3; }
 
 static int x12_step_mask(const omchat_ctx* ctx, int rows, int fmt) {
   if (rows != 1 || fmt != OMCHAT_WFMT_16 || ctx->dt != OMCHAT_BF16 || ctx->tp_size != 1) return 0;
-  return g_x12_roles & gemv_x12_default_forms();
+  const int forms = gemv_x12_default_forms();
+  return (g_x12_roles & forms) | ((g_x12_short & (forms >> omchat_ctx::X12_QKV)) << omchat_ctx::X12_QKV);
 }
 
 static int build_x12(omchat_ctx* ctx, int role) {
@@ -932,8 +935,9 @@
   if (T.state == omchat_ctx::W_BUILT || T.state == omchat_ctx::W_UNAVAILABLE) return 0;
   const omchat_config& c = ctx->c;
   const int H = c.t_hidden, It = c.t_mlp, L = c.t_layers;
-  const bool lm = role == omchat_ctx::X12_LM, down = role == omchat_ctx::X12_DOWN;
-  const size_t N = lm ? c.t_vocab : down ? H : 2 * (size_t)It, K = down ? It : H, n = lm ? 1 : L;
+  const bool lm = role == omchat_ctx::X12_LM, down = role == omchat_ctx::X12_DOWN, qkv = role == omchat_ctx::X12_QKV, op = role == omchat_ctx::X12_O;
+  const size_t N = lm ? c.t_vocab : (down || op) ? H : qkv ? ctx->t_qkvdim : 2 * (size_t)It, K = down ? It : op ? ctx->t_qdim : H, n = lm ? 1 : L;
+  const int proj = down ? omchat_ctx::P_DOWN : qkv ? omchat_ctx::P_QKV : op ? omchat_ctx::P_O : omchat_ctx::P_GU;
   const bool k_ok = K % 512 == 0 && (down ? (K > 4096 && K <= 32768) : K <= 4096);
   if (!k_ok || omchat_weights_missing(ctx) != 0) { if (!k_ok) T.state = omchat_ctx::W_UNAVAILABLE; return 0; }
   if (T.e.empty()) {
@@ -955,7 +959,7 @@
   OM_HIP(hipDeviceSynchronize());
   OM_HIP(hipMemset(ctx->x12_over, 0, n * 4));
   for (size_t j = 0; j < n; ++j) {
-    const void* W = lm ? ctx->lm_w(OMCHAT_WFMT_16).W : ctx->layer_w(OMCHAT_WFMT_16, (int)j)[down ? omchat_ctx::P_DOWN : omchat_ctx::P_GU].W;
+    const void* W = lm ? ctx->lm_w(OMCHAT_WFMT_16).W : ctx->layer_w(OMCHAT_WFMT_16, (int)j)[proj].W;
     const omchat_ctx::X12Ref& r = T.e[j];
     TRY(launch_encode_bf16x12(W, (int)K, (int)N, (int)K, r.W, r.top, r.cnt, r.patch, ctx->x12_over + j, nullptr));
   }
@@ -1419,6 +1423,7 @@
     if (n1) {
       GemvArgs g = gemv_args(x, H, W[QKV], H, ctx->tw_qkv, qkvd, 1, qkvd, L.bqkv, nullptr, EPI_NONE, 0, false);
       g.norm_w = L.ln1; g.norm_eps = c.t_eps;
+      if (const auto* r = x12_of(omchat_ctx::X12_QKV, i)) { use_weight_x12(g, *r, H); g.x12_short = 1; ++ctx->x12_launches[omchat_ctx::X12_QKV]; }
       if (OMCHAT_EXPERIMENTS && (g_ao_oproj & 16) && ctx->dbg_stamps) g.dbg = ctx->dbg_stamps + (size_t)i * 32;
       TRY(launch_gemv(ctx->dt, g, s));
     } else {
@@ -1480,6 +1485,12 @@
       GemvArgs g = gemv_args(ctx->tw_ao, qd, W16[O], qd, x, H, 1, H, nullptr, x, EPI_RESID, 0, false);
       g.dbg = ctx->dbg_stamps + (size_t)i * 32;
       TRY(launch_gemv(ctx->dt, g, s));
+    } else if (n2 && x12_of(omchat_ctx::X12_O, i)) {
+      GemvArgs g = gemv_args(ctx->tw_ao, qd, W[O], qd, x, H, 1, H, nullptr, x, EPI_RESID, 0, false);
+      use_weight_x12(g, *x12_of(omchat_ctx::X12_O, i), qd);
+      g.x12_short = 1;
+      ++ctx->x12_launches[omchat_ctx::X12_O];
+      TRY(launch_gemv(ctx->dt, g, s));
     } else if (n2) {
       TRY(gemv(ctx->tw_ao, qd, W[O], qd, x, H, H, nullptr, x, EPI_RESID));
     } else if (nb2) {
@@ -1592,11 +1603,22 @@
 extern "C" int omchat_bf16x12_stats(omchat_ctx* ctx, int* roles, long* launches, int* coded) {
   OM_CHECK(ctx, "null context");
   if (roles) *roles = g_x12_roles;
-  for (int r = 0; r < omchat_ctx::X12_ROLES; ++r) {
+  for (int r = 0; r < omchat_ctx::X12_LONG_ROLES; ++r) {
     if (launches) launches[r] = ctx->x12_launches[r];
     int n = 0;
     if (ctx->x12[r].state == omchat_ctx::W_BUILT) for (const auto& e : ctx->x12[r].e) n += e.ok ? 1 : 0;
     if (coded) coded[r] = n;
+  }
+  return 0;
+}
+extern "C" int omchat_bf16x12_short_stats(omchat_ctx* ctx, int* roles, long* launches, int* coded) {
+  OM_CHECK(ctx, "null context");
+  if (roles) *roles = g_x12_short;
+  for (int r = omchat_ctx::X12_QKV; r < omchat_ctx::X12_ROLES; ++r) {
+    if (launches) launches[r - omchat_ctx::X12_QKV] = ctx->x12_launches[r];
+    int n = 0;
+    if (ctx->x12[r].state == omchat_ctx::W_BUILT) for (const auto& e : ctx->x12[r].e) n += e.ok ? 1 : 0;
+    if (coded) coded[r - omchat_ctx::X12_QKV] = n;
   }
   return 0;
 }
diff --git a/omchat_amd/engine.py b/omchat_amd/engine.py
--- a/omchat_amd/engine.py
+++ b/omchat_amd/engine.py
@@ -186,6 +186,11 @@
         check(self.lib.omchat_bf16x12_stats(self.h, C.byref(roles), launches, coded))
         return dict(roles=roles.value, launches=list(launches), coded=list(coded))
 
+    def bf16x12_short_stats(self):
+        roles, launches, coded = C.c_int(0), (C.c_long * 2)(), (C.c_int * 2)()
+        check(self.lib.omchat_bf16x12_short_stats(self.h, C.byref(roles), launches, coded))
+        return dict(roles=roles.value, launches=list(launches), coded=list(coded))
+
     def prof_enable(self, on=True):
         check(self.lib.omchat_prof_enable(self.h, int(on)))
 
```

After: 393.8 (median of 5 runs). Within noise of the previous version (+0.6%).
